# zeal-up/ORB_SLAM_Tracking

Hardware: AMD Instinct MI355X
Metric: frames/sec (extract+match, 1000 feat, 640x480) (higher is better)
Workload: dtype u8

## Files before the change

### include/orbx.h

```cpp
#ifndef ORBX_H_
#define ORBX_H_

#include <stddef.h>
#include <stdint.h>

#ifdef __cplusplus
extern "C" {
#endif

#define ORBX_OK 0
#define ORBX_E_EMPTY (-1)
#define ORBX_E_BADARG (-2)
#define ORBX_E_TOOSMALL (-3)
#define ORBX_MAX_FRAME_DIM 4096
#define ORBX_E_HIP (-4)
#define ORBX_E_CAPACITY (-5)
#define ORBX_E_RCCL (-6)

typedef struct orbx_keypoint {
  float x, y, size, angle, response;
  int32_t octave, class_id;
} orbx_keypoint;

typedef struct orbx_params {
// ... 607 lines not shown
                                      const float* d_map_normals, const float* d_map_dist, const uint8_t* d_map_desc32,
                                      const uint8_t* d_map_mask, const float* d_pose, const float* K, const orbx_bounds* bounds,
                                      float th, float nnratio, int32_t* d_matches, const uint8_t* d_outlier, uint8_t* d_point_view,
                                      orbx_local_result* d_res);
int orbx_match_local_map(orbx_ctx* ctx, const orbx_keypoint* kps_un, const uint8_t* desc32, int n, int map_n,
                         const float* map_points, const float* map_normals, const float* map_dist, const uint8_t* map_desc32,
                         const uint8_t* map_mask, const float* pose, const float* K, const orbx_bounds* bounds, float th,
                         float nnratio, int32_t* matches, const uint8_t* outlier, uint8_t* point_view, orbx_local_result* res);

#define ORBX_KFPROJ_BAD_INPUT 2
#define ORBX_KFPROJ_NONFINITE 4
typedef struct orbx_kfproj_result {
  int32_t status;
  int32_t nmatches;
  int32_t n_points;
  int32_t n_found;
  int32_t n_behind_kept;
  int32_t n_out_image;
  int32_t n_out_distance;
  int32_t n_with_candidates;
  int32_t n_over_dist;
  int32_t n_displaced;
  int32_t n_rot_removed;
  int32_t n_outliers_cleared;
  int32_t rounds;
} orbx_kfproj_result;

int orbx_match_keyframe_projection_batch_device(orbx_ctx* ctx, int n_frames, int n_pairs, const int32_t* h_kf, const int32_t* h_cur,
                                                const int32_t* h_point_set, const orbx_keypoint* d_kps_un, const uint8_t* d_desc32,
                                                const int32_t* d_n, int capacity, int n_point_sets, const float* d_points,
                                                const uint8_t* d_point_mask, const uint8_t* d_point_desc32, const float* d_point_dist,
                                                const float* d_pose, const float* K, const orbx_bounds* bounds, float th, int orb_dist,
                                                int check_orientation, int32_t* d_matches, const uint8_t* d_outlier,
                                                orbx_kfproj_result* d_res);
int orbx_match_keyframe_projection(orbx_ctx* ctx, const orbx_keypoint* kf_kps_un, const uint8_t* kf_desc32, int kf_n,
                                   const orbx_keypoint* cur_kps_un, const uint8_t* cur_desc32, int cur_n, const float* points,
                                   const uint8_t* mask, const uint8_t* point_desc32, const float* point_dist, const float* pose,
                                   const float* K, const orbx_bounds* bounds, float th, int orb_dist, int check_orientation,
                                   int32_t* matches, const uint8_t* outlier, orbx_kfproj_result* res);

#define ORBX_MSIM3_BAD_INPUT 2
#define ORBX_MSIM3_NONFINITE 4
typedef struct orbx_msim3_result {
  int32_t status;
  int32_t n_found;
  int32_t n_points_12;
  int32_t n_behind_12;
  int32_t n_out_image_12;
  int32_t n_out_distance_12;
  int32_t n_with_candidates_12;
  int32_t n_over_dist_12;
  int32_t n_points_21, n_behind_21, n_out_image_21, n_out_distance_21, n_with_candidates_21, n_over_dist_21;
  int32_t n_one_sided;
  int32_t reserved;
} orbx_msim3_result;

int orbx_match_sim3_batch_device(orbx_ctx* ctx, int n_frames, int n_pairs, const int32_t* h_kf1, const int32_t* h_kf2,
                                 const int32_t* h_set1, const int32_t* h_set2, const orbx_keypoint* d_kps_un, const uint8_t* d_desc32,
                                 const int32_t* d_n, int capacity, int n_point_sets, const float* d_points,
                                 const uint8_t* d_point_mask, const uint8_t* d_point_desc32, const float* d_point_dist,
                                 const float* d_pose, const float* d_sim3, const float* K, const orbx_bounds* bounds, float th,
                                 int orb_dist, int32_t* d_matches, orbx_msim3_result* d_res);
int orbx_match_sim3(orbx_ctx* ctx, const orbx_keypoint* kps_un1, const uint8_t* desc1, int n1, const float* points1,
                    const uint8_t* mask1, const uint8_t* point_desc1, const float* point_dist1, const float* pose1,
                    const orbx_keypoint* kps_un2, const uint8_t* desc2, int n2, const float* points2, const uint8_t* mask2,
                    const uint8_t* point_desc2, const float* point_dist2, const float* pose2, const float* sim3, const float* K,
                    const orbx_bounds* bounds, float th, int orb_dist, int32_t* matches12, orbx_msim3_result* res);

#define ORBX_TRI_BAD_INPUT 2
#define ORBX_TRI_NONFINITE 4
#define ORBX_TRI_LOW_BASELINE 8
#define ORBX_TRI_ZERO_BASELINE 16
typedef struct orbx_tri_match_result {
  int32_t status;
  int32_t nmatches;
  int32_t n_queries;
  int32_t n_with_candidates;
  int32_t n_epipole_rejected;
  int32_t n_epiline_rejected;
  int32_t n_rot_removed;
  float baseline, ex, ey;
  float F12[9];
} orbx_tri_match_result;

int orbx_match_triangulation_batch_device(orbx_ctx* ctx, int n_frames, int n_pairs, const int32_t* h_kf1, const int32_t* h_kf2,
                                          const orbx_keypoint* d_kps_un, const uint8_t* d_desc32, const int32_t* d_n, int capacity,
                                          const uint32_t* d_fv_node, const uint32_t* d_fv_feat, const int32_t* d_fv_n,
                                          const uint8_t* d_mask, const float* d_pose, const float* K, const float* d_median_depth,
                                          int check_orientation, int32_t* d_matches12, orbx_tri_match_result* d_res);
int orbx_match_triangulation(orbx_ctx* ctx, const orbx_keypoint* kps_un1, const uint8_t* desc1, int n1, const uint32_t* fv_node1,
                             const uint32_t* fv_feat1, int fv_n1, const uint8_t* mask1, const float* pose1,
                             const orbx_keypoint* kps_un2, const uint8_t* desc2, int n2, const uint32_t* fv_node2,
                             const uint32_t* fv_feat2, int fv_n2, const uint8_t* mask2, const float* pose2, const float* K,
                             float median_depth2, int check_orientation, int32_t* matches12, orbx_tri_match_result* res);

typedef struct orbx_tri_result {
  int32_t status;
  int32_t n_matches;
  int32_t n_points;
  int32_t n_low_parallax, n_w_zero, n_behind_1, n_behind_2, n_reproj_1, n_reproj_2, n_zero_dist, n_scale;
} orbx_tri_result;

int orbx_triangulate_matches_batch_device(orbx_ctx* ctx, int n_frames, int n_pairs, const int32_t* h_kf1, const int32_t* h_kf2,
                                          const orbx_keypoint* d_kps_un, const int32_t* d_n, int capacity, const float* d_pose,
                                          const float* K, const int32_t* d_matches12, float* d_points, uint8_t* d_point_mask,
                                          float* d_point_normal, float* d_point_dist, orbx_tri_result* d_res);
int orbx_triangulate_matches(orbx_ctx* ctx, const orbx_keypoint* kps_un1, int n1, const float* pose1, const orbx_keypoint* kps_un2,
                             int n2, const float* pose2, const float* K, const int32_t* matches12, float* points, uint8_t* point_mask,
                             float* point_normal, float* point_dist, orbx_tri_result* res);

#define ORBX_STAGE_PYRAMID 0
#define ORBX_STAGE_FAST 1
#define ORBX_STAGE_SELECT 2
#define ORBX_STAGE_DESCRIBE 3
#define ORBX_STAGE_MATCH 4
#define ORBX_STAGE_COUNT 5
int orbx_profile_enable(orbx_ctx* ctx, int on);
int orbx_profile_stages(orbx_ctx* ctx, unsigned stage_mask);
int orbx_profile_reset(orbx_ctx* ctx);
int orbx_profile_get(orbx_ctx* ctx, double* ms, int64_t* launches);

typedef struct orbx_multi orbx_multi;
int orbx_multi_create(const orbx_params* params, int n_devices, const int* device_ids, int max_width, int max_height,
                      int max_batch_per_device, orbx_multi** out);
void orbx_multi_destroy(orbx_multi* m);
int orbx_multi_size(const orbx_multi* m);
orbx_ctx* orbx_multi_ctx(orbx_multi* m, int r);
const char* orbx_multi_last_error(const orbx_multi* m);
int orbx_multi_shard_range(int n_frames, int n_devices, int r, int* lo, int* hi);
int orbx_multi_extract_match_batch_device(orbx_multi* m, int n_frames, const uint8_t* const* d_imgs, int width, int height, int stride,
                                          size_t frame_stride_bytes, orbx_keypoint* const* d_kps, uint8_t* const* d_desc32, int capacity,
                                          int32_t* const* d_n_out, const orbx_bounds* bounds, int window_size, float nnratio,
                                          int check_orientation, int32_t* const* d_matches12, int32_t* const* d_nmatches,
                                          int32_t* counts_all);

int orbx_multi_set_pipeline_depth(orbx_multi* m, int depth);
int orbx_multi_extract_match_batch_device_async(orbx_multi* m, int n_frames, const uint8_t* const* d_imgs, int width, int height,
                                                int stride, size_t frame_stride_bytes, orbx_keypoint* const* d_kps,
                                                uint8_t* const* d_desc32, int capacity, int32_t* const* d_n_out,
                                                const orbx_bounds* bounds, int window_size, float nnratio, int check_orientation,
                                                int32_t* const* d_matches12, int32_t* const* d_nmatches, int32_t* counts_all);
int orbx_multi_wait_one(orbx_multi* m);
int orbx_multi_wait(orbx_multi* m);

int orbx_debug_candidates(orbx_ctx* ctx, int frame, int level, float* xyr, int cap);
int orbx_debug_selection_units(orbx_ctx* ctx, int frame, int32_t* counts, int32_t* redone);
int orbx_debug_distribute_device(orbx_ctx* ctx, const float* xyr, int n, int min_x, int max_x, int min_y, int max_y,
                                 int n_features, int variant, float* out_xyr, int cap);
int orbx_debug_std_sort(orbx_ctx* ctx, int32_t* triples, int n);
int orbx_debug_sincos(orbx_ctx* ctx, const float* angle_deg, int n, float* cos_out, float* sin_out);

int orbx_debug_last_launch(const orbx_ctx* ctx, int32_t* info8);
int orbx_debug_pyr_cols(int groups, int two_groups, uint32_t* info5);
int orbx_debug_match_counters(orbx_ctx* ctx, uint32_t* info4);
int orbx_debug_set(const char* key, long long value);
int orbx_debug_path_codes(int width, int height, int n, const int32_t* xs, const int32_t* ys, uint64_t* from_tables,
                          uint64_t* from_walk);

#ifdef __cplusplus
}
#endif
#endif
```

### orb_slam_tracking_amd/__init__.py

```python
from __future__ import annotations

import collections
import contextlib
import ctypes
import os
from typing import Optional, Sequence, Tuple

import numpy as np

__all__ = ["KEYPOINT_DTYPE", "OrbxError", "ORBextractor", "ORBmatcher", "Frame", "lib", "lib_path",
           "HFResult", "HF_RESULT_DTYPE", "Vocabulary", "BowResult", "BOW_MAX_FEATURES", "Database", "DB_MAX_RESULTS", "debug_database_shape", "InitResult", "INIT_RESULT_DTYPE", "BAResult", "BA_RESULT_DTYPE", "BA_SKIPPED", "BA_BAD_INPUT", "BA_NONFINITE", "BA_FEW_POINTS", "BA_NEGATIVE_DEPTH", "PoseResult", "POSE_RESULT_DTYPE", "POSE_BAD_INPUT", "POSE_NONFINITE", "POSE_FEW_POINTS", "PnpResult", "PNP_RESULT_DTYPE", "PNP_BAD_INPUT", "PNP_NONFINITE", "PNP_FEW_POINTS", "PNP_BAD_DRAWS", "PNP_NO_POSE", "PNP_RAND_MAX", "PnPsolver", "sample_pnp_draws", "Sim3Result", "SIM3_RESULT_DTYPE", "SIM3_BAD_INPUT", "SIM3_NONFINITE", "SIM3_FEW_POINTS", "SIM3_BAD_DRAWS", "SIM3_NO_RESULT", "Sim3Solver", "sample_sim3_draws", "MatchSim3Result", "MSIM3_RESULT_DTYPE", "MSIM3_BAD_INPUT", "MSIM3_NONFINITE", "ProjResult", "PROJ_RESULT_DTYPE", "PROJ_BAD_INPUT", "PROJ_NONFINITE", "LocalResult", "LOCAL_RESULT_DTYPE", "LOCAL_BAD_INPUT", "LOCAL_NONFINITE", "LOCAL_NOT_IN_VIEW", "LOCAL_SEEN", "KfProjResult", "KFPROJ_RESULT_DTYPE", "KFPROJ_BAD_INPUT", "KFPROJ_NONFINITE", "TriMatchResult", "TRI_MATCH_RESULT_DTYPE", "TriResult", "TRI_RESULT_DTYPE", "TRI_BAD_INPUT", "TRI_NONFINITE", "TRI_LOW_BASELINE", "TRI_ZERO_BASELINE", "Optimizer", "sample_sets", "INIT_TOO_FEW_MATCHES", "INIT_BAD_SETS", "INIT_NO_SCORE", "INIT_BAD_MATCHES",
           "STAGES", "E_EMPTY", "E_BADARG", "E_TOOSMALL", "E_HIP", "E_CAPACITY", "E_RCCL",
           "Sim3OptResult", "SIM3OPT_RESULT_DTYPE", "SIM3OPT_BAD_INPUT", "SIM3OPT_NONFINITE",
           "MatchScwResult", "SCW_RESULT_DTYPE", "SCW_BAD_INPUT", "SCW_NONFINITE", "SCW_TAKEN_UNMAPPED", "loop_accepted",
           "MapFuser", "FuseResult", "FUSE_RESULT_DTYPE", "FUSE_BAD_INPUT", "FUSE_NONFINITE", "FUSE_OCCUPIED_UNMAPPED", "FUSE_NONE",
           "FUSE_ADD", "FUSE_KEEP_OCCUPANT", "FUSE_REPLACE_OCCUPANT", "FUSE_BAD_OCCUPANT",
           "LbaResult", "LBA_RESULT_DTYPE", "LBA_BAD_INPUT", "LBA_NONFINITE", "LBA_MAX_FREE",
           "MapResult", "MAP_RESULT_DTYPE", "MAP_RESULT_FIELDS", "MAP_NORMALS", "MAP_DESCRIPTORS", "MAP_BAD_INPUT", "MAP_NONFINITE"]

from ._records import (KEYPOINT_DTYPE, _Params, _Bounds, _Camera, _Stats, HFResult, HF_RESULT_DTYPE, InitResult,
                       INIT_RESULT_DTYPE, BAResult, BA_RESULT_DTYPE, PoseResult, POSE_RESULT_DTYPE, PnpResult, PNP_RESULT_DTYPE,
                       Sim3Result, SIM3_RESULT_DTYPE, Sim3OptResult, SIM3OPT_RESULT_DTYPE, ProjResult, PROJ_RESULT_DTYPE,
                       PROJ_RESULT_FIELDS, LocalResult, LOCAL_RESULT_DTYPE, LOCAL_RESULT_FIELDS, MatchScwResult, SCW_RESULT_DTYPE,
                       SCW_RESULT_FIELDS, KfProjResult, KFPROJ_RESULT_DTYPE, KFPROJ_RESULT_FIELDS, MatchSim3Result,
# ... 131 lines not shown
    L.orbx_get_scale_factor.restype = f32
    L.orbx_get_tables.argtypes = [vp, vp, vp, vp, vp, vp]
    L.orbx_get_umax.argtypes = [vp, vp]
    L.orbx_extract.argtypes = [vp, vp, i32, i32, i32, i32, i32, vp, vp, i32, vp]
    L.orbx_host_register.argtypes = [vp, vp, sz]
    L.orbx_host_unregister.argtypes = [vp, vp]
    L.orbx_extract_batch.argtypes = [vp, i32, vp, i32, i32, i32, sz, i32, i32, vp, vp, i32, vp, vp]
    L.orbx_extract_batch_device.argtypes = [vp, i32, vp, i32, i32, i32, sz, vp, vp, i32, vp]
    L.orbx_level_size.argtypes = [vp, i32, vp, vp]
    L.orbx_download_pyramid.argtypes = [vp, i32, i32, i32, vp, i32]
    L.orbx_match_init.argtypes = [vp, vp, vp, i32, vp, vp, i32, ctypes.POINTER(_Bounds), i32, f32, i32, vp,
                                  ctypes.POINTER(ctypes.c_int32), ctypes.POINTER(_Stats)]
    L.orbx_match_init_batch_device.argtypes = [vp, i32, vp, vp, vp, vp, vp, i32, ctypes.POINTER(_Bounds), i32, f32, i32,
                                               vp, vp, vp]
    L.orbx_extract_match_batch_device.argtypes = [vp, i32, vp, i32, i32, i32, sz, vp, vp, i32, vp, i32, vp, vp,
                                                  ctypes.POINTER(_Bounds), i32, f32, i32, vp, vp, vp]
    L.orbx_extract_match_batch_device_async.argtypes = [vp, i32, vp, i32, i32, i32, sz, vp, vp, i32, vp, i32, vp, vp,
                                                  ctypes.POINTER(_Bounds), i32, f32, i32, vp, vp, vp]
    L.orbx_extract_match_batch_host_async.argtypes = L.orbx_extract_match_batch_device_async.argtypes
    L.orbx_set_opencv_variant.argtypes = [vp, i32, i32]
    L.orbx_set_libm_variant.argtypes = [vp, i32]
    L.orbx_set_pipeline_depth.argtypes = [vp, i32]
    L.orbx_wait_one.argtypes = [vp]
    L.orbx_wait.argtypes = [vp]
    L.orbx_order_after.argtypes = [vp, vp]
    L.orbx_order_before.argtypes = [vp, vp]
    L.orbx_profile_stages.argtypes = [vp, ctypes.c_uint]
    L.orbx_undistort_keypoints.argtypes = [vp, vp, i32, ctypes.POINTER(_Camera), vp]
    L.orbx_undistort_batch_device.argtypes = [vp, i32, vp, vp, i32, ctypes.POINTER(_Camera), vp]
    L.orbx_image_bounds.argtypes = [vp, ctypes.POINTER(_Camera), i32, i32, ctypes.POINTER(_Bounds)]
    L.orbx_to_gray.argtypes = [vp, vp, i32, i32, i32, i32, i32, vp, i32]
    L.orbx_to_gray_batch_device.argtypes = [vp, i32, vp, i32, i32, i32, sz, i32, i32, vp, i32, sz]
    L.orbx_check_homography.argtypes = [vp, i32, vp, vp, vp, i32, vp, i32, vp, f32, vp, vp, vp, vp]
    L.orbx_check_fundamental.argtypes = [vp, i32, vp, vp, i32, vp, i32, vp, f32, vp, vp, vp, vp]
    L.orbx_check_rt.argtypes = [vp, i32, vp, vp, vp, vp, i32, vp, i32, vp, vp, f32, vp, vp, vp, vp]
    L.orbx_find_models_batch_device.argtypes = [vp, i32, i32, vp, vp, vp, vp, i32, vp, i32, vp, f32, vp, vp, vp, vp]
    L.orbx_find_models.argtypes = [vp, vp, i32, vp, i32, vp, i32, vp, f32, ctypes.POINTER(HFResult), vp, vp, vp]
    L.orbx_initialize_batch_device.argtypes = [vp, i32, i32, vp, vp, vp, vp, i32, vp, i32, vp, vp, f32, f32, i32, vp, vp, vp]
    L.orbx_initialize.argtypes = [vp, vp, i32, vp, i32, vp, i32, vp, vp, f32, f32, i32, ctypes.POINTER(InitResult), vp, vp]
    L.orbx_bundle_adjust_batch_device.argtypes = [vp, i32, i32, vp, vp, vp, vp, i32, vp, vp, vp, vp, vp, vp, i32, i32, i32, vp, vp]
    L.orbx_bundle_adjust.argtypes = [vp, vp, i32, vp, i32, vp, vp, vp, vp, vp, vp, i32, i32, i32, ctypes.POINTER(BAResult), vp]
    L.orbx_pose_optimize_batch_device.argtypes = [vp, i32, i32, vp, vp, vp, vp, i32, vp, i32, vp, vp, vp, vp, vp, i32, vp, vp]
    L.orbx_pose_optimize.argtypes = [vp, vp, i32, vp, vp, vp, vp, vp, i32, ctypes.POINTER(PoseResult), vp]
    f64 = ctypes.c_double
    L.orbx_pnp_ransac_table.argtypes = [f64, i32, i32, f32, i32, vp]
    L.orbx_pnp_solve_batch_device.argtypes = [vp, i32, i32, vp, vp, vp, vp, i32, vp, i32, vp, vp, vp, vp, f64, i32, i32, f32, f32, i32,
                                              vp, vp, vp, vp, vp]
    L.orbx_pnp_solve.argtypes = [vp, vp, i32, vp, vp, vp, vp, f64, i32, i32, f32, f32, i32, vp, ctypes.POINTER(PnpResult), vp]
    L.orbx_sim3_ransac_table.argtypes = [f64, i32, i32, i32, vp]
    L.orbx_sim3_solve_batch_device.argtypes = [vp, i32, i32, vp, vp, vp, vp, vp, vp, i32, vp, i32, vp, vp, vp, vp, vp, i32, f64, i32, i32,
                                               f32, i32, vp, vp, vp, vp, vp]
    L.orbx_match_sim3_batch_device.argtypes = [vp, i32, i32, vp, vp, vp, vp, vp, vp, vp, i32, i32, vp, vp, vp, vp, vp, vp, vp,
                                               ctypes.POINTER(_Bounds), f32, i32, vp, vp]
    L.orbx_match_sim3.argtypes = [vp, vp, vp, i32, vp, vp, vp, vp, vp, vp, vp, i32, vp, vp, vp, vp, vp, vp, vp, ctypes.POINTER(_Bounds),
                                  f32, i32, vp, ctypes.POINTER(MatchSim3Result)]
    L.orbx_sim3_solve.argtypes = [vp, vp, i32, vp, vp, vp, vp, i32, vp, vp, vp, vp, vp, vp, i32, f64, i32, i32, f32, i32, vp,
                                  ctypes.POINTER(Sim3Result), vp, vp, vp]
    L.orbx_optimize_sim3_batch_device.argtypes = [vp, i32, i32, vp, vp, vp, vp, vp, vp, i32, vp, i32, vp, vp, vp, vp, vp, vp, i32, f32,
                                                  i32, i32, vp, vp]
    L.orbx_optimize_sim3.argtypes = [vp, vp, i32, vp, vp, vp, vp, i32, vp, vp, vp, vp, vp, vp, vp, i32, f32, i32, i32,
                                     ctypes.POINTER(Sim3OptResult), vp]
    L.orbx_match_scw_batch_device.argtypes = [vp, i32, i32, vp, vp, vp, vp, vp, i32, i32, i32, vp, vp, vp, vp, vp, vp, vp, vp,
                                              ctypes.POINTER(_Bounds), f32, i32, vp, vp, vp]
    L.orbx_match_scw.argtypes = [vp, vp, vp, i32, i32, vp, vp, vp, vp, vp, vp, vp, ctypes.POINTER(_Bounds), f32, i32, vp, vp, i32,
                                 ctypes.POINTER(MatchScwResult)]
    L.orbx_sim3_compose_scw_batch_device.argtypes = [vp, i32, i32, vp, vp, vp, vp]
    L.orbx_sim3_compose_scw.argtypes = [vp, vp, vp, vp]
    L.orbx_fuse_batch_device.argtypes = [vp, i32, i32, vp, vp, vp, vp, vp, i32, i32, i32, vp, vp, vp, vp, vp, vp, vp, vp, vp,
                                         ctypes.POINTER(_Bounds), f32, i32, vp, vp, vp, vp, vp, vp]
    L.orbx_fuse_scw_batch_device.argtypes = [vp, i32, i32, vp, vp, vp, vp, vp, i32, i32, i32, vp, vp, vp, vp, vp, vp, vp, vp,
                                             ctypes.POINTER(_Bounds), f32, i32, vp, vp, vp, vp, vp, vp]
    L.orbx_fuse.argtypes = [vp, vp, vp, i32, i32, vp, vp, vp, vp, vp, vp, vp, vp, ctypes.POINTER(_Bounds), f32, i32, vp, vp, vp, vp, vp,
                            ctypes.POINTER(FuseResult)]
    L.orbx_fuse_scw.argtypes = [vp, vp, vp, i32, i32, vp, vp, vp, vp, vp, vp, vp, ctypes.POINTER(_Bounds), f32, i32, vp, vp, vp, vp, vp,
                                ctypes.POINTER(FuseResult)]
    L.orbx_local_ba_batch_device.argtypes = [vp, i32, i32, vp, vp, vp, vp, i32, vp, vp, vp, i32, vp, vp, i32, i32, vp, vp, vp, vp, vp, i32, i32,
                                             vp, vp, vp, vp]
    L.orbx_local_ba.argtypes = [vp, i32, i32, vp, vp, i32, vp, vp, i32, vp, vp, vp, vp, i32, i32, vp, vp, vp, ctypes.POINTER(LbaResult)]
    L.orbx_debug_local_ba_lds_max_free.argtypes = [i32]
    L.orbx_map_update_batch_device.argtypes = [vp, i32, i32, vp, vp, vp, vp, i32, vp, vp, vp, vp, i32, vp, vp, vp, i32, i32, vp, vp, vp, vp, vp,
                                               i32, vp, vp, vp, vp, vp]
    L.orbx_map_update.argtypes = [vp, i32, i32, vp, vp, vp, i32, vp, vp, vp, i32, vp, vp, vp, vp, i32, vp, vp, vp, vp, ctypes.POINTER(MapResult)]
    L.orbx_vocabulary_parse_text.argtypes = [ctypes.c_char_p, vp, vp, vp, vp, vp, vp, i32]
    L.orbx_vocabulary_create.argtypes = [vp, i32, i32, i32, i32, i32, vp, vp, vp, vp, ctypes.POINTER(vp)]
    L.orbx_vocabulary_load_text.argtypes = [vp, ctypes.c_char_p, ctypes.POINTER(vp)]
    L.orbx_vocabulary_destroy.argtypes = [vp]
    L.orbx_vocabulary_destroy.restype = None
    L.orbx_vocabulary_info.argtypes = [vp, vp]
    L.orbx_vocabulary_get_nodes.argtypes = [vp, vp, vp, vp, vp, i32]
    L.orbx_vocabulary_save_text.argtypes = [vp, ctypes.c_char_p, i32]
    L.orbx_vocabulary_train_device.argtypes = [vp, i32, i32, i32, i32, ctypes.c_uint64, i32, i32, vp, vp, i32, ctypes.POINTER(vp), vp, vp]
    L.orbx_vocabulary_train.argtypes = [vp, i32, i32, i32, i32, ctypes.c_uint64, i32, i32, vp, vp, ctypes.POINTER(vp), vp, vp]
    L.orbx_debug_voc_train_seed_grid_min.argtypes = [ctypes.c_longlong]
    L.orbx_bow_transform_batch_device.argtypes = [vp, vp, i32, vp, vp, i32, i32, vp, vp, vp, vp, vp, vp, vp]
    L.orbx_bow_transform.argtypes = [vp, vp, vp, i32, i32, vp, vp, vp, vp, vp, vp, vp]
    L.orbx_bow_score_batch_device.argtypes = [vp, vp, i32, i32, vp, vp, vp, vp, vp, i32, vp]
    L.orbx_bow_score.argtypes = [vp, vp, vp, vp, i32, vp, vp, i32, vp]
    L.orbx_match_bow_batch_device.argtypes = [vp, i32, i32, vp, vp, vp, vp, vp, i32, vp, vp, vp, vp, f32, i32, vp, vp]
    L.orbx_match_bow.argtypes = [vp, vp, vp, i32, vp, vp, i32, vp, vp, i32, vp, vp, i32, vp, f32, i32, vp, vp]
    L.orbx_match_projection_batch_device.argtypes = [vp, i32, i32, vp, vp, vp, vp, vp, vp, i32, i32, vp, vp, vp, vp, vp, vp,
                                                     ctypes.POINTER(_Bounds), f32, i32, vp, vp]
    L.orbx_match_projection.argtypes = [vp, vp, vp, i32, vp, vp, i32, vp, vp, vp, vp, vp, vp, ctypes.POINTER(_Bounds), f32, i32, vp,
                                        ctypes.POINTER(ProjResult)]
    L.orbx_match_local_map_batch_device.argtypes = [vp, i32, i32, vp, vp, vp, vp, vp, i32, i32, i32, vp, vp, vp, vp, vp, vp, vp, vp,
                                                    ctypes.POINTER(_Bounds), f32, f32, vp, vp, vp, vp]
    L.orbx_match_local_map.argtypes = [vp, vp, vp, i32, i32, vp, vp, vp, vp, vp, vp, vp, ctypes.POINTER(_Bounds), f32, f32, vp, vp, vp,
                                       ctypes.POINTER(LocalResult)]
    L.orbx_match_keyframe_projection_batch_device.argtypes = [vp, i32, i32, vp, vp, vp, vp, vp, vp, i32, i32, vp, vp, vp, vp, vp, vp,
                                                              ctypes.POINTER(_Bounds), f32, i32, i32, vp, vp, vp]
    L.orbx_match_keyframe_projection.argtypes = [vp, vp, vp, i32, vp, vp, i32, vp, vp, vp, vp, vp, vp, ctypes.POINTER(_Bounds), f32,
                                                 i32, i32, vp, vp, ctypes.POINTER(KfProjResult)]
    L.orbx_match_triangulation_batch_device.argtypes = [vp, i32, i32, vp, vp, vp, vp, vp, i32, vp, vp, vp, vp, vp, vp, vp, i32, vp, vp]
    L.orbx_match_triangulation.argtypes = [vp, vp, vp, i32, vp, vp, i32, vp, vp, vp, vp, i32, vp, vp, i32, vp, vp, vp, f32, i32, vp,
                                           ctypes.POINTER(TriMatchResult)]
    L.orbx_triangulate_matches_batch_device.argtypes = [vp, i32, i32, vp, vp, vp, vp, i32, vp, vp, vp, vp, vp, vp, vp, vp]
    L.orbx_triangulate_matches.argtypes = [vp, vp, i32, vp, vp, i32, vp, vp, vp, vp, vp, vp, vp, ctypes.POINTER(TriResult)]
    L.orbx_database_create.argtypes = [vp, vp, ctypes.POINTER(vp)]
    L.orbx_database_destroy.argtypes = [vp]
    L.orbx_database_destroy.restype = None
    L.orbx_database_clear.argtypes = [vp]
    L.orbx_database_size.argtypes = [vp]
    L.orbx_database_add_batch_device.argtypes = [vp, vp, i32, vp, vp, vp, i32, vp]
    L.orbx_database_query_batch_device.argtypes = [vp, vp, i32, vp, vp, vp, i32, i32, i32, vp, vp, vp]
    L.orbx_database_add.argtypes = [vp, vp, vp, vp, i32, vp]
    L.orbx_database_query.argtypes = [vp, vp, vp, vp, i32, i32, i32, vp, vp, vp]
    L.orbx_database_get_inverted_file.argtypes = [vp, vp, vp, vp, ctypes.c_int64]
    L.orbx_database_get_inverted_file.restype = ctypes.c_int64
    L.orbx_debug_database_shape.argtypes = [i32, i32]
    L.orbx_multi_create.argtypes = [ctypes.POINTER(_Params), i32, vp, i32, i32, i32, ctypes.POINTER(vp)]
    L.orbx_multi_destroy.argtypes = [vp]
    L.orbx_multi_destroy.restype = None
    L.orbx_multi_size.argtypes = [vp]
    L.orbx_multi_ctx.argtypes = [vp, i32]
    L.orbx_multi_ctx.restype = vp
    L.orbx_multi_last_error.argtypes = [vp]
    L.orbx_multi_last_error.restype = ctypes.c_char_p
    L.orbx_multi_shard_range.argtypes = [i32, i32, i32, ctypes.POINTER(i32), ctypes.POINTER(i32)]
    L.orbx_multi_extract_match_batch_device.argtypes = [vp, i32, vp, i32, i32, i32, sz, vp, vp, i32, vp, ctypes.POINTER(_Bounds), i32,
                                                        f32, i32, vp, vp, vp]
    L.orbx_multi_extract_match_batch_device_async.argtypes = L.orbx_multi_extract_match_batch_device.argtypes
    L.orbx_multi_set_pipeline_depth.argtypes = [vp, i32]
    L.orbx_multi_wait_one.argtypes = [vp]
    L.orbx_multi_wait.argtypes = [vp]
    L.orbx_profile_enable.argtypes = [vp, i32]
    L.orbx_profile_reset.argtypes = [vp]
    L.orbx_profile_get.argtypes = [vp, vp, vp]
    L.orbx_debug_candidates.argtypes = [vp, i32, i32, vp, i32]
    L.orbx_debug_distribute_device.argtypes = [vp, vp, i32, i32, i32, i32, i32, i32, i32, vp, i32]
    L.orbx_debug_std_sort.argtypes = [vp, vp, i32]
    L.orbx_debug_sincos.argtypes = [vp, vp, i32, vp, vp]
    L.orbx_debug_set.argtypes = [ctypes.c_char_p, ctypes.c_longlong]
    L.orbx_debug_last_launch.argtypes = [vp, vp]
    L.orbx_debug_pyr_cols.argtypes = [ctypes.c_int, ctypes.c_int, vp]
    L.orbx_debug_match_counters.argtypes = [vp, vp]
    L.orbx_debug_selection_units.argtypes = [vp, i32, vp, vp]
    L.orbx_debug_path_codes.argtypes = [ctypes.c_int, ctypes.c_int, ctypes.c_int, vp, vp, vp, vp]
    _LIB = L
    for name in KNOBS:
        v = os.environ.get("ORBX_" + name.upper())
        if v is not None:
            debug_set(name, _knob_value(name, v))
    return L


KNOBS = ("no_bands", "pyr_bands", "pyr_strips", "bands_min_frames", "no_split", "lat_trace", "fast_wg_max_cells", "match_no_general",
         "match_no_mfma", "oct_big_depth", "oct_big_no_fallback", "multi_force_rccl")
KNOB_UNSET = -(1 << 63)


def _knob_value(name: str, text: str) -> int:
    try:
        return int(text)
    except ValueError:
        return 1


def debug_set(name: str, value: Optional[int]) -> None:
    r = lib().orbx_debug_set(name.encode(), KNOB_UNSET if value is None else int(value))
    if r != 0:
        raise OrbxError(r, "orbx_debug_set(%r)" % name)


@contextlib.contextmanager
def knobs(**values: Optional[int]):
    try:
        for name, value in values.items():
            debug_set(name, value)
        yield
    finally:
        for name in values:
            debug_set(name, None)


def _ptr(a) -> ctypes.c_void_p:
    if a is None:
        return ctypes.c_void_p(0)
    if isinstance(a, np.ndarray):
        return ctypes.c_void_p(a.ctypes.data)
    if hasattr(a, "data_ptr"):
        return ctypes.c_void_p(a.data_ptr())
    return ctypes.c_void_p(int(a))


def _nbytes(a):
    if isinstance(a, np.ndarray):
        return int(a.nbytes)
    if hasattr(a, "data_ptr") and hasattr(a, "numel"):
        return int(a.numel()) * int(a.element_size())
    return None


def _need(what: str, a, nbytes: int) -> None:
    have = _nbytes(a)
    if have is not None and have < nbytes:
        raise ValueError("%s holds %d bytes, the call needs %d" % (what, have, nbytes))


def _pair_lists(names, lists, n_frames: Optional[int] = None, n_sets: Optional[int] = None, set_what: str = "") -> list:
    rows = [np.ascontiguousarray(a, np.int32).reshape(-1) for a in lists]
    n = len(rows[0])
    for r in rows:
        if len(r) != n:
            raise OrbxError(E_BADARG, "%s and %s must have the same length" % (", ".join(names[:-1]), names[-1]))
    if n and (n_frames is not None or n_sets is not None):
        top = [int(r.view(np.uint32).max()) for r in rows]
        if n_frames is not None and max(top if n_sets is None else top[:-1]) >= n_frames:
            raise ValueError("a pair names a frame outside the batch of %d" % n_frames)
        if n_sets is not None and top[-1] >= n_sets:
            raise ValueError("a pair names a %s outside the %d given" % (set_what, n_sets))
    return rows


def _k9(K) -> np.ndarray:
    return np.ascontiguousarray(K, np.float32).reshape(9)


def _bounds(bounds) -> _Bounds:
    return _Bounds(*[int(v) for v in bounds])


def _keys(keys) -> np.ndarray:
    return np.ascontiguousarray(keys, KEYPOINT_DTYPE).reshape(-1)


def _desc(desc, n: Optional[int] = None, message: str = "") -> Optional[np.ndarray]:
    if desc is None and n is not None:
        return None
    d = np.ascontiguousarray(desc, np.uint8).reshape(-1, 32)
    if n is not None and len(d) != n:
        raise OrbxError(E_BADARG, message)
    return d


def _points(points, width: int = 3) -> np.ndarray:
    return np.ascontiguousarray(points, np.float32).reshape(-1, width)


def _flags(flags, n: int, message: str) -> Optional[np.ndarray]:
    if flags is None:
        return None
    f = np.ascontiguousarray(np.asarray(flags) != 0, np.uint8).reshape(-1)
    if len(f) != n:
        raise OrbxError(E_BADARG, message)
    return f


def _row(row, n: int, message: str) -> np.ndarray:
    out = np.full(max(n, 1), -1, np.int32)
    if row is not None:
        given = np.asarray(row, np.int32).reshape(-1)
        if len(given) != n:
            raise OrbxError(E_BADARG, message)
        out[:n] = given
    return out


def _per_level(table, nlevels: int, name: str) -> Optional[np.ndarray]:
    t = None if table is None else np.ascontiguousarray(table, np.float32)
    if t is not None and len(t) != nlevels:
        raise OrbxError(E_BADARG, "%s must have one entry per pyramid level" % name)
    return t


def _pose12(Tcw) -> np.ndarray:
    T = np.asarray(Tcw, np.float32)
    if T.ndim == 1:
        return np.ascontiguousarray(T.reshape(12))
    return np.ascontiguousarray(np.r_[T[:3, :3].reshape(9), T[:3, 3]], np.float32)


def _camera_K(K, holder, who: str, what: str = "frame") -> np.ndarray:
    if K is not None:
        return K
    cam = getattr(holder, "camera", None)
    if cam is None:
        raise OrbxError(E_BADARG, "%s needs K (the %s carries no camera)" % (who, what))
    return np.array([[cam[0], 0, cam[2]], [0, cam[1], cam[3]], [0, 0, 1]], np.float32)


def _need_batch(imgs, n_frames, width, height, stride, frame_stride, kps, desc, n, capacity, first=None, second=None, matches12=None,
                nmatches=None, stats=None, init_res=None, p3d=None, triangulated=None, ba_res=None, p3d_out=None) -> None:
    if n_frames > 0 and imgs is not None:
        _need("the frames", imgs, (n_frames - 1) * frame_stride + (height - 1) * stride + width)
    _need("the keypoint array", kps, n_frames * capacity * 28)
    _need("the descriptor array", desc, n_frames * capacity * 32)
    _need("the count array", n, n_frames * 4)
# ... 1907 lines not shown
```

### orb_slam_tracking_amd/csrc/orbx_api.cpp

```cpp
#include <hip/hip_runtime.h>

#include <algorithm>
#include <cmath>
#include <cstdio>
#include <cstring>
#include <ctime>
#include <string>
#include <vector>

#include "orbx_host.h"
#include "orbx_knobs.h"

namespace orbx {

std::atomic<long long> g_knob[KNOB_COUNT] = {
#define ORBX_KNOB_INIT(e, n) {KNOB_UNSET},
    ORBX_KNOB_LIST(ORBX_KNOB_INIT)
#undef ORBX_KNOB_INIT
};

namespace {

inline int cvRoundF(float v) { return (int)lrintf(v); }
inline int cvRoundD(double v) { return (int)lrint(v); }

}
}

using namespace orbx;

struct PyrTabInfo {
  int32_t xoff[ORBX_MAX_LEVELS], yoff[ORBX_MAX_LEVELS];
  int ok, dual2;
};

struct SizedBufs {
  DeviceBuf<uint8_t> dPyr;
  DeviceBuf<uint32_t> dCand;
  DeviceBuf<int> dCandCount;
  DeviceBuf<int> dCellCount;
  DeviceBuf<int> dMaxN;
  PinnedBuf<int> hMaxN;
  DeviceBuf<ResizeTab> dTab;
  DeviceBuf<FastCell> dCells;
  DeviceBuf<SelKp> dSel;
  DeviceBuf<int> dNsel;
  DeviceBuf<SelKp> dSelStage;
  DeviceBuf<int> dNselLevel;
  DeviceBuf<uint8_t> dOctScratch;
  DeviceBuf<uint32_t> dOctTab;
  DeviceBuf<PyrTileRect> dPyrTiles;
  DeviceBuf<PyrTileTap> dPyrTaps;
  DeviceBuf<uint8_t> dIn;
  DeviceBuf<orbx_keypoint> dKps;
  DeviceBuf<uint8_t> dDesc;
  PinnedBuf<int> hNsel;
  PinnedBuf<int> hFlags;
  PinnedBuf<int> hWide;
  PinnedBuf<orbx_keypoint> hKpsPin;
  PinnedBuf<uint8_t> hDescPin;
};

struct PairBlock {
  orbx_keypoint* kps = nullptr;
  uint8_t* desc = nullptr;
  int32_t* n = nullptr;
  size_t bytes = 0;
  PairBlock() = default;
  PairBlock(void* base, size_t cap) {
    Layout L(base);
    kps = L.take<orbx_keypoint>(2 * cap);
    desc = L.take<uint8_t>(2 * cap * 32);
    n = L.take<int32_t>(2);
    bytes = L.size();
  }
};

struct orbx_ctx {
  orbx_params p{};
  int device = 0;
  hipStream_t st = nullptr;
  bool ownStream = false;
  int maxW = 0, maxH = 0, maxB = 0;
  std::vector<float> scale, invScale, sigma2, invSigma2;
  std::vector<int> quota;
  int umax[16]{};
  int gaussVariant = 0, grayVariant = 0;
  int libmVariant = ORBX_LIBM_DEFAULT;
  int selCap = 0;

  int curW = 0, curH = 0, curStride0 = 0;
  Geom g{};
  std::vector<ResizeTab> hTab;

  SizedBufs bufs;
  size_t pyrBytes = 0;
  size_t candEntries = 0;
  int candHintL[ORBX_MAX_LEVELS]{};
  int maxSlotsUsed = 0;
  size_t cellCountEntries = 0;
  size_t tabEntries = 0;
  PyrTabInfo pyrInfo{};
  std::vector<FastCell> hCells;
  size_t cellEntries = 0;
  int fastWaveOk = 0;
  OctLaunch oct{};
  int maxQuota = 0;
  size_t pyrTileCap = 0;
  std::vector<PyrTileRect> hPyrTiles;
  std::vector<PyrTileTap> hPyrTaps;
  int nPyrTiles = 0, pyrTileBuf0 = 0, pyrTileBuf = 0;
  size_t octTabEntries = 0;
  std::vector<uint32_t> hOctTab;
  size_t octScratchBytes = 0;
  bool wideExpected = false;
  int wideIdle = 0;
  bool wideLaunched[2]{};
  bool eventOrdered = false;
  int lastLaunch[8]{};
  struct LateMatch {
    bool valid = false;
    int nPairs = 0, capacity = 0, window = 0, checkOri = 0;
    float nnratio = 0;
    orbx_bounds b{};
    const orbx_keypoint* dKps = nullptr;
    const uint8_t* dDesc = nullptr;
    const int* dN = nullptr;
    int32_t* dMatches12 = nullptr;
    int32_t* dNmatches = nullptr;
    int32_t* dStats = nullptr;
  } late[2];
  size_t inBytes = 0;
  int pinFrames = 0;
  DeviceBuf<int> dMatchScratch;
  DeviceBuf<unsigned int> dMatchDiag;
  HeldArray<int32_t> pairs;
  DeviceBuf<uint8_t> dMblk;
  PinnedBuf<uint8_t> hMblk;
  PairBlock dM, hM;
  PinnedBuf<int> hMo;
  DeviceBuf<int> dMi;
  size_t mCap = 0;
  DeviceBuf<uint8_t> io;
  InitScratch init;
  DeviceBuf<uint8_t> dColor;
  MatchBowScratch matchBow;
  BaScratch ba;
  PoseScratch pose;
  PnpScratch pnp;
  Sim3Scratch sim3;
  Sim3OptScratch sim3Opt;
  LbaScratch lba;
  MapScratch map;
  TriScratch tri;

  const uint8_t* lastImg0 = nullptr;
  long long lastFrameStride0 = 0;
  int lastB = 0;

  hipStream_t st2 = nullptr;
  hipEvent_t evFork = nullptr, evJoin = nullptr;
  hipEvent_t evOrder = nullptr;

  unsigned profMask = 0;
  hipEvent_t ev[2][2][ORBX_STAGE_COUNT][2]{};
  bool used[2][2][ORBX_STAGE_COUNT]{};
  hipEvent_t evDone[2]{};
  hipEvent_t evDone2[2]{};
  bool done2Used[2]{};
  std::vector<orbx_ctx*> lanes;
  unsigned laneIssue = 0, laneDone = 0;
  bool noSplit = false;
  DeviceBuf<uint8_t> dPipeOut;
  hipEvent_t evOut[2]{};
  bool outUsed[2]{};
  bool hostInput = false;
  unsigned seqIssue = 0;
  int pending = 0;
  int parity = 0;
  double ms[ORBX_STAGE_COUNT]{};
  int64_t launches[ORBX_STAGE_COUNT]{};

  std::string err;
};

namespace {

void computeTables(orbx_ctx* c) {
  const int nl = c->p.nlevels;
  const double scaleFactor = (double)c->p.scale_factor;
  c->scale.assign(nl, 1.f);
  c->sigma2.assign(nl, 1.f);
  c->invScale.assign(nl, 1.f);
  c->invSigma2.assign(nl, 1.f);
  for (int i = 1; i < nl; i++) {
    c->scale[i] = (float)(c->scale[i - 1] * scaleFactor);
    c->sigma2[i] = c->scale[i] * c->scale[i];
  }
  for (int i = 0; i < nl; i++) {
    c->invScale[i] = 1.0f / c->scale[i];
    c->invSigma2[i] = 1.0f / c->sigma2[i];
  }
  c->quota.assign(nl, 0);
  const float factor = (float)(1.0f / scaleFactor);
  const float powv = c->libmVariant ? powf(factor, (float)nl) : (float)std::pow((double)factor, (double)(float)nl);
  float desired = c->p.nfeatures * (1 - factor) / (1 - powv);
  int sum = 0;
  for (int l = 0; l < nl - 1; l++) {
    c->quota[l] = cvRoundF(desired);
    sum += c->quota[l];
    desired *= factor;
  }
  c->quota[nl - 1] = std::max(c->p.nfeatures - sum, 0);
  c->selCap = 0;
  for (int q : c->quota) c->selCap += q;
  const int HALF = 15;
  const int vmax = (int)std::floor(HALF * std::sqrt(2.f) / 2 + 1);
  const int vmin = (int)std::ceil(HALF * std::sqrt(2.f) / 2);
  const double hp2 = HALF * HALF;
  for (int v = 0; v <= HALF; v++) c->umax[v] = 0;
  for (int v = 0; v <= vmax; ++v) c->umax[v] = cvRoundD(std::sqrt(hp2 - v * v));
  for (int v = HALF, v0 = 0; v >= vmin; --v) {
    while (c->umax[v0] == c->umax[v0 + 1]) ++v0;
    c->umax[v] = v0;
    ++v0;
  }
}

void levelSize(const orbx_ctx* c, int w, int h, int l, int* lw, int* lh) {
  *lw = cvRoundF(w * c->invScale[l]);
  *lh = cvRoundF(h * c->invScale[l]);
}

void appendPyrTables(const Geom& g, std::vector<ResizeTab>* tab, PyrTabInfo* info) {
  static_assert(sizeof(ResizeTab) == 8 && sizeof(PyrXGroup) == 8 * sizeof(ResizeTab) && sizeof(PyrYRow) == 2 * sizeof(ResizeTab), "table units");
  *info = PyrTabInfo{};
  info->ok = g.nlevels > 1;
  for (int l = 1; l < g.nlevels; l++) {
    const LevelGeom& S = g.L[l - 1];
    const LevelGeom& D = g.L[l];
    const int sw = S.w, sh = S.h, ng = (D.w + 3) / 4;
    if (sw < 8 || D.h >= 32768 || D.w > 4096) info->ok = 0;
    if (tab->size() & 1) tab->push_back(ResizeTab{0, 0});
    info->xoff[l] = (int32_t)(tab->size() / 2);
    const int lim = (sw - 1) & ~3;
    for (int gx = 0; gx < ng; gx++) {
      PyrXGroup x{};
      const ResizeTab* e = tab->data() + D.xtabOff + 4 * gx;
      const int base = e[0].ofs & ~3;
      x.o[0] = (uint32_t)base;
      x.o[1] = (uint32_t)std::min(base + 4, lim);
      x.o[2] = (uint32_t)std::min(base + 8, lim);
      const uint32_t zero = 0x0c0c0c0cu;
      for (int i = 0; i < 4; i++) {
        const int k = e[i].ofs - base, c0 = e[i].coef & 0xffff, c1 = (int)((uint32_t)e[i].coef >> 16);
        const int k1 = c1 ? k + 1 : k;
        if (k < 0 || k1 > 11 || c0 + c1 > 2048) { info->ok = 0; continue; }
        const bool second = k1 > 7;
        if (second && k < 4) { info->ok = 0; continue; }
        const uint32_t sel = 0x0c000c00u | (uint32_t)(second ? k - 4 : k) | ((uint32_t)(second ? k1 - 4 : k1) << 16);
        if (i < 2) {
          if (second) info->ok = 0;
          x.sel[i] = sel;
        } else if (i == 2) {
          x.sel[2] = second ? zero : sel;
          x.sel[3] = second ? sel : zero;
          if (second) info->dual2 = 1;
        } else {
          x.sel[4] = second ? zero : sel;
          x.sel[5] = second ? sel : zero;
        }
        x.cf[i] = ((uint32_t)c0 << 4) | (((uint32_t)c1 << 4) << 16);
      }
      ResizeTab raw[8];
      memcpy(raw, &x, sizeof(x));
      tab->insert(tab->end(), raw, raw + 8);
    }
    info->yoff[l] = (int32_t)(tab->size() / 2);
    for (int dy = 0; dy < D.h; dy++) {
      const ResizeTab t = (*tab)[D.ytabOff + dy];
      const int sy0 = std::min(std::max(t.ofs, 0), sh - 1), sy1 = std::min(std::max(t.ofs + 1, 0), sh - 1);
      const int c0 = t.coef & 0xffff, c1 = (int)((uint32_t)t.coef >> 16);
      if (c0 + c1 > 2048) info->ok = 0;
      const PyrYRow y{(uint32_t)sy0 * (uint32_t)S.stride, (uint32_t)sy1 * (uint32_t)S.stride, (uint32_t)c0 << 8, (uint32_t)c1 << 8};
      ResizeTab raw[2];
      memcpy(raw, &y, sizeof(y));
      tab->insert(tab->end(), raw, raw + 2);
    }
  }
}

int buildGeometry(orbx_ctx* c, int w, int h, int stride0, Geom* out, std::vector<ResizeTab>* tab, PyrTabInfo* pyrInfo = nullptr) {
  Geom g{};
  g.nlevels = c->p.nlevels;
  g.iniTh = std::min(std::max(c->p.ini_th_fast, 0), 255);
  g.minTh = std::min(std::max(c->p.min_th_fast, 0), 255);
  g.selCap = c->selCap;
  int cellBase = 0;
  int64_t pyrOff = 0, candOff = 0;
  int tabOff = 0;
  if (tab) tab->clear();
  int pw = 0, ph = 0;
  for (int l = 0; l < g.nlevels; l++) {
    LevelGeom& L = g.L[l];
    levelSize(c, w, h, l, &L.w, &L.h);
    if (L.w > ORBX_MAX_FRAME_DIM || L.h > ORBX_MAX_FRAME_DIM) {
      c->err = "frame larger than ORBX_MAX_FRAME_DIM (4096) pixels in width or height";
      return ORBX_E_BADARG;
    }
    L.maxBX = L.w - ORBX_EDGE + 3;
    L.maxBY = L.h - ORBX_EDGE + 3;
    const float width = (float)(L.maxBX - ORBX_MIN_BORDER), height = (float)(L.maxBY - ORBX_MIN_BORDER);
    if (width < 35.f || height < 35.f) return ORBX_E_TOOSMALL;
    if ((int)std::round(width / height) < 1) return ORBX_E_TOOSMALL;
    L.nCols = (int)(width / 35.f);
    L.nRows = (int)(height / 35.f);
    L.wCell = (int)std::ceil(width / L.nCols);
    L.hCell = (int)std::ceil(height / L.nRows);
    L.cellBase = cellBase;
    L.colsInv24 = L.nCols > 0 ? (uint32_t)(((1u << 24) + (uint32_t)L.nCols - 1u) / (uint32_t)L.nCols) : 0u;
    cellBase += L.nCols * L.nRows;
    int cap = 0;
    for (int i = 0; i < L.nRows; i++) {
      const int iniY = ORBX_MIN_BORDER + i * L.hCell;
      if (iniY >= L.maxBY - 3) continue;
      const int ch = std::min(iniY + L.hCell + 6, L.maxBY) - iniY;
      for (int j = 0; j < L.nCols; j++) {
        const int iniX = ORBX_MIN_BORDER + j * L.wCell;
        if (iniX >= L.maxBX - 6) continue;
        const int cw = std::min(iniX + L.wCell + 6, L.maxBX) - iniX;
        if (cw < 7 || ch < 7) continue;
        cap += ((cw - 6 + 1) / 2) * ((ch - 6 + 1) / 2);
      }
    }
    L.candMax = std::max(cap, 1);
    L.segCap = alignUp(std::max(((L.wCell + 1) / 2) * ((L.hCell + 1) / 2), 1), 4);
    L.candCap = L.nCols * L.nRows * L.segCap;
    L.candOff = candOff;
    candOff += (int64_t)L.candCap * c->maxB;
    L.quota = c->quota[l];
    L.scale = c->scale[l];
    L.patchSize = (int)(31 * c->scale[l]);
    if (l == 0) {
      L.stride = stride0;
      L.imgOff = 0;
      L.frameStride = 0;
      L.xtabOff = L.ytabOff = 0;
    } else {
      L.stride = alignUp(L.w, 64);
      L.imgOff = pyrOff;
      L.frameStride = (int64_t)L.stride * L.h;
      pyrOff += L.frameStride * c->maxB;
      if (tab) {
        const int sw = pw, sh = ph, dw = L.w, dh = L.h;
        const double scale_x = 1.0 / ((double)dw / sw), scale_y = 1.0 / ((double)dh / sh);
        L.xtabOff = tabOff;
        const int dwPad = alignUp(dw, 4);
        for (int dx = 0; dx < dwPad; dx++) {
          const int d = std::min(dx, dw - 1);
          float fx = (float)((d + 0.5) * scale_x - 0.5);
          int sx = (int)std::floor(fx);
          fx -= sx;
          if (sx < 0) { fx = 0; sx = 0; }
          if (sx >= sw - 1) { fx = 0; sx = sw - 1; }
          const int c0 = cvRoundF((1.f - fx) * 2048), c1 = cvRoundF(fx * 2048);
          tab->push_back(ResizeTab{sx, (c0 & 0xffff) | (c1 << 16)});
        }
        int span = 0;
        for (int dx = 0; dx + 3 < dwPad; dx += 4)
          span = std::max(span, (*tab)[L.xtabOff + dx + 3].ofs - (*tab)[L.xtabOff + dx].ofs);
        L.resizeSpanOk = span <= 7 ? 1 : 0;
        tabOff += dwPad;
        L.ytabOff = tabOff;
        for (int dy = 0; dy < dh; dy++) {
          float fy = (float)((dy + 0.5) * scale_y - 0.5);
          int sy = (int)std::floor(fy);
          fy -= sy;
          const int c0 = cvRoundF((1.f - fy) * 2048), c1 = cvRoundF(fy * 2048);
          tab->push_back(ResizeTab{sy, (c0 & 0xffff) | (c1 << 16)});
        }
        tabOff += dh;
      }
    }
    pw = L.w;
    ph = L.h;
  }
  g.nCellsTotal = cellBase;
  if (tab) {
    PyrTabInfo info;
    appendPyrTables(g, tab, &info);
    if (pyrInfo) *pyrInfo = info;
  }
  *out = g;
  return ORBX_OK;
}

int buildFastCells(const Geom& g, std::vector<FastCell>* out) {
  out->assign((size_t)g.nCellsTotal, FastCell{});
  bool ok = true, narrow = true;
  for (int l = 0; l < g.nlevels; l++) {
    const LevelGeom& L = g.L[l];
    for (int ci = 0; ci < L.nRows; ci++)
      for (int cj = 0; cj < L.nCols; cj++) {
        const int local = ci * L.nCols + cj;
        FastCell& c = (*out)[(size_t)L.cellBase + local];
        c.xoff_level = (uint32_t)l << 16;
        c.stride = (uint32_t)L.stride;
        c.segOff = (uint32_t)local * (uint32_t)L.segCap;
        c.segCap = (uint32_t)L.segCap;
        const int iniY = ORBX_MIN_BORDER + ci * L.hCell, iniX = ORBX_MIN_BORDER + cj * L.wCell;
        if (iniY >= L.maxBY - 3 || iniX >= L.maxBX - 6) continue;
        const int maxY = std::min(iniY + L.hCell + 6, L.maxBY), maxX = std::min(iniX + L.wCell + 6, L.maxBX);
        const int cw = maxX - iniX, ch = maxY - iniY;
        if (cw < 7 || ch < 7) continue;
        const int ax0 = iniX & ~3, xoff = iniX - ax0, nw = (maxX - ax0 + 3) >> 2;
        if (nw > 16 || ch > 64) ok = false;
        if (nw > 12) narrow = false;
        c.imgOff = (uint32_t)(iniY * L.stride + ax0);
        c.nw_ch = (uint32_t)nw | ((uint32_t)ch << 16);
        c.iw_ih = (uint32_t)(cw - 6) | ((uint32_t)(ch - 6) << 16);
        c.xoff_level |= (uint32_t)xoff;
        c.ox_oy = ((uint32_t)(cj * L.wCell - xoff) & 0xffffu) | ((uint32_t)(ci * L.hCell) << 16);
      }
  }
  return ok ? (narrow ? 2 : 1) : 0;
}

struct Sizes {
  size_t pyrBytes, candEntries, tabEntries;
};
Sizes sizesOf(const orbx_ctx* c, const Geom& g, size_t tabEntries) {
  Sizes s{};
  const LevelGeom& last = g.L[g.nlevels - 1];
  s.pyrBytes = g.nlevels > 1 ? (size_t)(last.imgOff + last.frameStride * c->maxB) : 0;
  s.candEntries = (size_t)(last.candOff + (int64_t)last.candCap * c->maxB);
  s.tabEntries = tabEntries;
  return s;
}

int octDepthBits(int height, float hX) {
  int e = std::max((int)std::ceil(hX) + 1, height), d = 0;
  while (e > 1) { e = (e + 1) >> 1; d++; }
  return std::max(d, 1);
}

constexpr long long kPyrTilesMaxPixels = 2500000ll;
void pyrTileGrid(const Geom& g, int* TX, int* TY) {
  *TX = std::max(1, (g.L[1].w + 35) / 36);
  *TY = std::max(1, (g.L[1].h + 27) / 28);
}
bool buildPyrTiles(const Geom& g, const std::vector<ResizeTab>& tab, std::vector<PyrTileRect>* out, std::vector<PyrTileTap>* taps,
                   int* nTiles, int* buf0Bytes, int* bufBytes) {
  const int nl = g.nlevels;
  *nTiles = 0;
  *buf0Bytes = *bufBytes = 0;
  out->clear();
  taps->clear();
  if (nl < 2 || g.L[0].w > 32000 || g.L[0].h > 32000) return false;
  int TX, TY;
  pyrTileGrid(g, &TX, &TY);
  out->assign((size_t)TX * TY * nl, PyrTileRect{});
  taps->assign((size_t)TX * TY * ORBX_PYR_TILE_TAPS, PyrTileTap{0, 0});
  int maxPix = 0, maxPix0 = 0;
  for (int tj = 0; tj < TY; tj++)
    for (int ti = 0; ti < TX; ti++) {
      PyrTileRect* R = out->data() + (size_t)(tj * TX + ti) * nl;
      for (int l = 1; l < nl; l++) {
        R[l].ox0 = (int16_t)((long long)ti * g.L[l].w / TX); R[l].ox1 = (int16_t)((long long)(ti + 1) * g.L[l].w / TX);
        R[l].oy0 = (int16_t)((long long)tj * g.L[l].h / TY); R[l].oy1 = (int16_t)((long long)(tj + 1) * g.L[l].h / TY);
      }
      for (int l = nl - 1; l >= 0; l--) {
        int x0 = R[l].ox0, x1 = R[l].ox1, y0 = R[l].oy0, y1 = R[l].oy1;
        const bool ownEmpty = x1 <= x0 || y1 <= y0;
        if (l + 1 < nl && R[l + 1].nx1 > R[l + 1].nx0 && R[l + 1].ny1 > R[l + 1].ny0) {
          const ResizeTab* xt = tab.data() + g.L[l + 1].xtabOff;
          const ResizeTab* yt = tab.data() + g.L[l + 1].ytabOff;
          const int w = g.L[l].w, h = g.L[l].h;
          const int fx0 = std::min(std::max(xt[R[l + 1].nx0].ofs, 0), w - 1), fx1 = std::min(xt[R[l + 1].nx1 - 1].ofs + 1, w - 1) + 1;
          const int fy0 = std::min(std::max(yt[R[l + 1].ny0].ofs, 0), h - 1);
          const int fy1 = std::min(std::max(yt[R[l + 1].ny1 - 1].ofs + 1, 0), h - 1) + 1;
          if (ownEmpty) { x0 = fx0; x1 = fx1; y0 = fy0; y1 = fy1; }
          else { x0 = std::min(x0, fx0); x1 = std::max(x1, fx1); y0 = std::min(y0, fy0); y1 = std::max(y1, fy1); }
        } else if (ownEmpty) {
          x0 = x1 = y0 = y1 = 0;
        }
        R[l].nx0 = (int16_t)x0; R[l].nx1 = (int16_t)x1; R[l].ny0 = (int16_t)y0; R[l].ny1 = (int16_t)y1;
        (l == 0 ? maxPix0 : maxPix) = std::max(l == 0 ? maxPix0 : maxPix, (x1 - x0) * (y1 - y0));
        if ((long long)(x1 - x0) * (y1 - y0) * (x1 - x0) >= (1ll << 20)) { out->clear(); taps->clear(); return false; }
      }
      PyrTileTap* T = taps->data() + (size_t)(tj * TX + ti) * ORBX_PYR_TILE_TAPS;
      int nT = 0;
      for (int l = 1; l < nl; l++) {
        const ResizeTab* xt = tab.data() + g.L[l].xtabOff;
        const ResizeTab* yt = tab.data() + g.L[l].ytabOff;
        const int sw = g.L[l - 1].w, sh = g.L[l - 1].h;
        const int nw = R[l].nx1 - R[l].nx0, nh = R[l].ny1 - R[l].ny0;
        if (nT + nw + nh > ORBX_PYR_TILE_TAPS) { out->clear(); taps->clear(); return false; }
        for (int x = R[l].nx0; x < R[l].nx1; x++) {
          const int sx = xt[x].ofs, sx1 = std::min(sx + 1, sw - 1);
          T[nT++] = PyrTileTap{(uint32_t)(sx - R[l - 1].nx0) | ((uint32_t)(sx1 - sx) << 16), (uint32_t)xt[x].coef};
        }
        for (int y = R[l].ny0; y < R[l].ny1; y++) {
          const int sy0 = std::min(std::max(yt[y].ofs, 0), sh - 1), sy1 = std::min(std::max(yt[y].ofs + 1, 0), sh - 1);
          T[nT++] = PyrTileTap{(uint32_t)(sy0 - R[l - 1].ny0) | ((uint32_t)(sy1 - sy0) << 16), (uint32_t)yt[y].coef};
        }
      }
    }
  const int buf0 = (maxPix0 + 63) & ~63, buf = (maxPix + 63) & ~63;
  if (buf0 <= 0 || buf <= 0 || ORBX_PYR_TILE_TAPS * (int)sizeof(PyrTileTap) + buf0 + 2 * buf > 60 * 1024) { out->clear(); taps->clear(); return false; }
  *nTiles = TX * TY;
  *buf0Bytes = buf0;
  *bufBytes = buf;
  return true;
}

void octCodeTable(const OctLevel& O, uint32_t* out) {
  for (int xi = 0; xi < O.tabW; xi++) {
    const float x = (float)xi;
    int root = (int)(x / O.hX);
    root = std::min(std::max(root, 0), O.nIni - 1);
    int ul = (int)(O.hX * (float)root), br = (int)(O.hX * (float)(root + 1));
    uint32_t s = 0;
    for (int d = 0; d < 16; d++) {
      const int mid = ul + ((br - ul + 1) >> 1);
      const uint32_t q = !(x < (float)mid);
      if (q) ul = mid; else br = mid;
      s = (s << 2) | q;
    }
    out[2 * xi] = s;
    out[2 * xi + 1] = (uint32_t)root;
  }
  uint32_t* ty = out + 2 * (size_t)O.tabW;
  for (int yi = 0; yi < O.tabH; yi++) {
    const float y = (float)yi;
    int ul = 0, br = O.height;
    uint32_t s = 0;
    for (int d = 0; d < 16; d++) {
      const int mid = ul + ((br - ul + 1) >> 1);
      const uint32_t q = !(y < (float)mid);
      if (q) ul = mid; else br = mid;
      s = (s << 2) | (q << 1);
    }
    ty[yi] = s;
  }
}
void octBigPlan(OctLevel* O, int nMax) {
  O->bigDMax = -1;
  O->bigD0 = 0; O->bigBuckets = 0; O->bigCapB = 0;
  if (O->nIni < 1 || O->nIni > ORBX_OCTB_MAX_BUCKETS || O->quota < 1) return;
  int kq = 0;
  while ((long long)O->nIni << (2 * (kq + 1)) <= (long long)O->quota && kq < 8) kq++;
  int d = kq;
  while (d > 0 && ((long long)O->nIni << (2 * d)) > ORBX_OCTB_MAX_BUCKETS) d--;
  O->bigDMax = d;
  octBigChoose(O, nMax, 0);
}
inline size_t octBigTabDwords(const OctLevel& O) {
  return O.bigDMax >= 0 ? ((size_t)O.nIni << O.bigDMax) + 1 + ((size_t)1 << O.bigDMax) + 1 : 0;
}
size_t octTabLayout(OctLaunch* P) {
  size_t off = 0;
  for (int l = 0; l < P->nlevels; l++) {
    OctLevel& O = P->lev[l];
    O.tabOff = (int32_t)off;
    off += (2 * (size_t)O.tabW + (size_t)O.tabH + 1) & ~(size_t)1;
    O.bigTabOff = (int32_t)off;
    off += (octBigTabDwords(O) + 1) & ~(size_t)1;
  }
  return off;
}
bool octBigTable(const OctLevel& O, const uint32_t* codeTab, uint32_t* out) {
  const int d0 = O.bigDMax, nx = O.nIni << d0, ny = 1 << d0;
  auto topBits = [&](uint32_t s, int odd) {
    uint32_t v = 0;
    for (int d = 1; d <= d0; d++) v = (v << 1) | ((s >> (2 * (16 - d) + odd)) & 1u);
    return v;
  };
  std::vector<int> first((size_t)std::max(nx, ny) + 1);
// ... 1511 lines not shown

int orbx_debug_selection_units(orbx_ctx* ctx, int frame, int32_t* counts, int32_t* redone) {
  if (!ctx || frame < 0 || frame >= ctx->lastB || !counts) return ORBX_E_BADARG;
  if (hipSetDevice(ctx->device) != hipSuccess) return ORBX_E_HIP;
  {
    const int w = waitAll(ctx);
    if (w == ORBX_E_HIP) return w;
  }
  const int nl = ctx->p.nlevels;
  std::vector<int32_t> raw((size_t)nl);
  HIPCHK(hipMemcpy(raw.data(), ctx->bufs.dNselLevel + (size_t)frame * nl, sizeof(int32_t) * (size_t)nl, hipMemcpyDeviceToHost));
  for (int l = 0; l < nl; l++) {
    counts[l] = raw[l] < 0 ? raw[l] : (raw[l] & ~ORBX_OCT_REDONE);
    if (redone) redone[l] = raw[l] >= 0 && (raw[l] & ORBX_OCT_REDONE) ? 1 : 0;
  }
  return ORBX_OK;
}

}

extern "C" {

int orbx_debug_distribute_device(orbx_ctx* ctx, const float* xyr, int n, int min_x, int max_x, int min_y, int max_y,
                                 int n_features, int variant, float* out_xyr, int cap) {
  if (!ctx || n < 0 || (n > 0 && !xyr) || max_x <= min_x || max_y <= min_y || n_features < 0 || n > ORBX_OCT_MAX_CAND)
    return ORBX_E_BADARG;
  if (hipSetDevice(ctx->device) != hipSuccess) return ORBX_E_HIP;
  OctLaunch P{};
  P.nlevels = 1;
  P.selStride = std::max(n_features, 1);
  OctLevel& O = P.lev[0];
  O.width = max_x - min_x;
  O.height = max_y - min_y;
  O.nIni = (int)std::round((float)O.width / (float)O.height);
  if (O.nIni < 1 || O.nIni > 255) return ORBX_E_TOOSMALL;
  O.hX = (float)O.width / (float)O.nIni;
  O.depthBits = octDepthBits(O.height, O.hX);
  O.tabW = O.tabH = 4096;
  O.wCell = O.hCell = 1 << 20;
  O.nCols = 1;
  O.quota = n_features;
  O.cellBase = 0; O.nCells = 1; O.segCap = alignUp(std::max(n, 1), 4);
  P.nCellsTotal = 1;
  P.candCap[0] = std::max(n, 1);
  P.scrNMax[0] = std::min(std::max(8 * n, 16384), ORBX_OCT_MAX_CAND);
  P.scrStride[0] = (int64_t)octScratchBytes(P.scrNMax[0], std::max(n_features, O.nIni));
  std::vector<uint32_t> packed((size_t)alignUp(std::max(n, 1), 4));
  for (int i = 0; i < n; i++) {
    const int x = (int)xyr[3 * i], y = (int)xyr[3 * i + 1], r = (int)xyr[3 * i + 2];
    if (x < 0 || x > 4095 || y < 0 || y > 4095 || r < 0 || r > 255) return ORBX_E_BADARG;
    packed[i] = packCand(x, y, r);
  }
  O.tabW = std::max(O.tabW, O.width);
  O.tabH = std::max(O.tabH, O.height);
  octBigPlan(&O, P.scrNMax[0]);
  octTabLayout(&P);
  std::vector<uint32_t> codeTab;
  octCodeTables(&P, &codeTab);
  std::vector<SelKp> sel(std::max(n_features, 1));
  int res[2] = {0, 0};
  DeviceBuf<uint32_t> dC, dT;
  DeviceBuf<int> dI;
  DeviceBuf<SelKp> dS;
  DeviceBuf<uint8_t> dScr;
  HIPCHK(dC.grow(packed.size() * 4));
  HIPCHK(dI.grow(2 * sizeof(int)));
  HIPCHK(dS.grow(sel.size() * sizeof(SelKp)));
  HIPCHK(dScr.grow((size_t)P.scrStride[0]));
  HIPCHK(dT.grow(codeTab.size() * 4));
  P.codeTab = dT;
  HIPCHK(hipMemcpyAsync(dT, codeTab.data(), codeTab.size() * 4, hipMemcpyHostToDevice, ctx->st));
  HIPCHK(hipMemcpyAsync(dC, packed.data(), packed.size() * 4, hipMemcpyHostToDevice, ctx->st));
  int hi[2] = {n, -7};
  HIPCHK(hipMemcpyAsync(dI, hi, sizeof hi, hipMemcpyHostToDevice, ctx->st));
  const int hintN[ORBX_MAX_LEVELS] = {n};
  HIPCHK(launch_octree(ctx->st, 1, dC, dI, P, dS, dI + 1, dScr, nullptr, variant == 5 ? hintN : nullptr,
                       variant == 1 ? -1 : variant == 2 ? 1024 : variant == 3 ? 512 : variant == 4 ? (2048 | 0x10000) : variant == 5 ? -2 :
                       variant == 6 ? -3 : 0, nullptr));
  HIPCHK(hipMemcpyAsync(res, dI, sizeof res, hipMemcpyDeviceToHost, ctx->st));
  HIPCHK(hipMemcpyAsync(sel.data(), dS, sel.size() * sizeof(SelKp), hipMemcpyDeviceToHost, ctx->st));
  HIPCHK(hipStreamSynchronize(ctx->st));
  if (res[1] < 0) return ORBX_E_CAPACITY;
  res[1] &= ~0x40000000;
  for (int i = 0; i < res[1] && i < cap; i++) {
    out_xyr[3 * i] = (float)(sel[i].x - ORBX_MIN_BORDER);
    out_xyr[3 * i + 1] = (float)(sel[i].y - ORBX_MIN_BORDER);
    out_xyr[3 * i + 2] = (float)sel[i].response;
  }
  return res[1];
}

int orbx_debug_path_codes(int width, int height, int n, const int32_t* xs, const int32_t* ys, uint64_t* from_tables,
                          uint64_t* from_walk) {
  if (width <= 0 || height <= 0 || width > 4096 || height > 4096 || n < 0 || (n > 0 && (!xs || !ys || !from_tables || !from_walk)))
    return ORBX_E_BADARG;
  OctLevel O{};
  O.width = width;
  O.height = height;
  O.nIni = (int)std::round((float)width / (float)height);
  if (O.nIni < 1 || O.nIni > 255) return ORBX_E_TOOSMALL;
  O.hX = (float)width / (float)O.nIni;
  O.tabW = width;
  O.tabH = height;
  std::vector<uint32_t> tab((size_t)2 * width + height + 2);
  octCodeTable(O, tab.data());
  for (int i = 0; i < n; i++) {
    const int xi = xs[i], yi = ys[i];
    if (xi < 0 || xi >= width || yi < 0 || yi >= height) return ORBX_E_BADARG;
    from_tables[i] = ((uint64_t)tab[2 * (size_t)xi + 1] << 32) | (uint64_t)(tab[2 * (size_t)xi] | tab[2 * (size_t)width + yi]);
    const float x = (float)xi, y = (float)yi;
    int root = (int)(x / O.hX);
    root = std::min(std::max(root, 0), O.nIni - 1);
    int ulx = (int)(O.hX * (float)root), brx = (int)(O.hX * (float)(root + 1)), uly = 0, bry = height;
    uint64_t code = (uint64_t)root;
    for (int d = 0; d < 16; d++) {
      const int midX = ulx + ((brx - ulx + 1) >> 1), midY = uly + ((bry - uly + 1) >> 1);
      const int qx = !(x < (float)midX), qy = !(y < (float)midY);
      if (qx) ulx = midX; else brx = midX;
      if (qy) uly = midY; else bry = midY;
      code = (code << 2) | (uint64_t)(qy * 2 + qx);
    }
    from_walk[i] = code;
  }
  return ORBX_OK;
}

int orbx_debug_set(const char* key, long long value) {
  static const char* const names[KNOB_COUNT] = {
#define ORBX_KNOB_NAME(e, n) n,
      ORBX_KNOB_LIST(ORBX_KNOB_NAME)
#undef ORBX_KNOB_NAME
  };
  if (!key) return ORBX_E_BADARG;
  for (int k = 0; k < KNOB_COUNT; k++)
    if (std::strcmp(key, names[k]) == 0) {
      g_knob[k].store(value, std::memory_order_relaxed);
      return ORBX_OK;
    }
  return ORBX_E_BADARG;
}

int orbx_debug_pyr_cols(int groups, int two_groups, uint32_t* info5) {
  if (!info5 || groups < 1 || groups > (two_groups ? 2 : 1) * ORBX_PYR_THREADS) return ORBX_E_BADARG;
  uint32_t c[2];
  pyrColsOf(groups, two_groups != 0, c);
  info5[0] = (c[0] >> 31) + 1;
  info5[1] = (c[0] >> 20 & 0x1ffu) + 1;
  info5[2] = (c[1] >> 20 & 0x1ffu) + 1;
  info5[3] = c[0] & 0xfffffu;
  info5[4] = c[1] & 0xfffffu;
  return ORBX_OK;
}

int orbx_debug_last_launch(const orbx_ctx* ctx, int32_t* info8) {
  if (!ctx || !info8) return ORBX_E_BADARG;
  for (int i = 0; i < 8; i++) info8[i] = ctx->lastLaunch[i];
  return ORBX_OK;
}

int orbx_debug_match_counters(orbx_ctx* ctx, uint32_t* info4) {
  if (!ctx || !info4) return ORBX_E_BADARG;
  for (int i = 0; i < 4; i++) info4[i] = 0;
  if (!ctx->dMatchDiag) return ORBX_OK;
  if (hipSetDevice(ctx->device) != hipSuccess) return ORBX_E_HIP;
  const int w = waitAll(ctx);
  if (w != ORBX_OK) return w;
  HIPCHK(hipStreamSynchronize(ctx->st));
  HIPCHK(hipMemcpy(info4, ctx->dMatchDiag, 4 * sizeof(uint32_t), hipMemcpyDeviceToHost));
  return ORBX_OK;
}

int orbx_debug_sincos(orbx_ctx* ctx, const float* angle_deg, int n, float* cos_out, float* sin_out) {
  if (!ctx || n < 0 || (n > 0 && (!angle_deg || !cos_out || !sin_out))) return ORBX_E_BADARG;
  if (n == 0) return ORBX_OK;
  if (hipSetDevice(ctx->device) != hipSuccess) return ORBX_E_HIP;
  DeviceBuf<float> d;
  HIPCHK(d.grow((size_t)n * 3 * sizeof(float)));
  HIPCHK(hipMemcpyAsync(d, angle_deg, (size_t)n * sizeof(float), hipMemcpyHostToDevice, ctx->st));
  HIPCHK(launch_debug_sincos(ctx->st, d, n, d + n, d + 2 * (size_t)n, ctx->libmVariant));
  HIPCHK(hipMemcpyAsync(cos_out, d + n, (size_t)n * sizeof(float), hipMemcpyDeviceToHost, ctx->st));
  HIPCHK(hipMemcpyAsync(sin_out, d + 2 * (size_t)n, (size_t)n * sizeof(float), hipMemcpyDeviceToHost, ctx->st));
  HIPCHK(hipStreamSynchronize(ctx->st));
  return ORBX_OK;
}

int orbx_debug_std_sort(orbx_ctx* ctx, int32_t* triples, int n) {
  if (!ctx || n < 0 || (n > 0 && !triples)) return ORBX_E_BADARG;
  if (n == 0) return ORBX_OK;
  if (hipSetDevice(ctx->device) != hipSuccess) return ORBX_E_HIP;
  DeviceBuf<int> d;
  DeviceBuf<unsigned long long> w;
  HIPCHK(d.grow((size_t)n * 3 * sizeof(int)));
  HIPCHK(w.grow((size_t)n * 2 * sizeof(unsigned long long)));
  HIPCHK(hipMemcpyAsync(d, triples, (size_t)n * 3 * sizeof(int), hipMemcpyHostToDevice, ctx->st));
  HIPCHK(launch_debug_sort(ctx->st, d, n, w, w + n));
  HIPCHK(hipMemcpyAsync(triples, d, (size_t)n * 3 * sizeof(int), hipMemcpyDeviceToHost, ctx->st));
  HIPCHK(hipStreamSynchronize(ctx->st));
  return ORBX_OK;
}

}

namespace orbx {
int ctxDevice(const orbx_ctx* c) { return c->device; }
hipStream_t ctxStream(const orbx_ctx* c) { return c->st; }
int ctxDrain(orbx_ctx* c) {
  if (hipSetDevice(c->device) != hipSuccess) return ORBX_E_HIP;
  return waitAll(c);
}
void ctxSetError(orbx_ctx* c, const char* msg) { c->err = msg; }
DeviceBuf<uint8_t>& ctxIo(orbx_ctx* c) { return c->io; }
InitScratch* ctxInit(orbx_ctx* c) { return &c->init; }
MatchBowScratch* ctxMatchBow(orbx_ctx* c) { return &c->matchBow; }
BaScratch* ctxBa(orbx_ctx* c) { return &c->ba; }
PoseScratch* ctxPose(orbx_ctx* c) { return &c->pose; }
PnpScratch* ctxPnp(orbx_ctx* c) { return &c->pnp; }
Sim3Scratch* ctxSim3(orbx_ctx* c) { return &c->sim3; }
Sim3OptScratch* ctxSim3Opt(orbx_ctx* c) { return &c->sim3Opt; }
LbaScratch* ctxLba(orbx_ctx* c) { return &c->lba; }
MapScratch* ctxMap(orbx_ctx* c) { return &c->map; }
TriScratch* ctxTri(orbx_ctx* c) { return &c->tri; }
const float* ctxInvSigma2(const orbx_ctx* c, int* nlevels) {
  *nlevels = c->p.nlevels;
  return c->invSigma2.data();
}
const float* ctxSigma2(const orbx_ctx* c, int* nlevels) {
  *nlevels = c->p.nlevels;
  return c->sigma2.data();
}
const float* ctxScale(const orbx_ctx* c, int* nlevels) {
  *nlevels = c->p.nlevels;
  return c->scale.data();
}
}
```

### orb_slam_tracking_amd/csrc/orbx_device.h

```cpp
#pragma once
#include <algorithm>
#include <cstdint>

#include "../../include/orbx.h"

#define ORBX_MAX_LEVELS 16
#define ORBX_EDGE 19
#define ORBX_MIN_BORDER 16
#define ORBX_CELL_MAX 76
#define ORBX_GRID_COLS 64
#define ORBX_GRID_ROWS 48

namespace orbx {

struct LevelGeom {
  int32_t w, h, stride;
  int32_t nCols, nRows;
  int32_t wCell, hCell;
  int32_t maxBX, maxBY;
  int32_t cellBase;
  int32_t candCap;
  int32_t quota;
  int32_t xtabOff, ytabOff;
  int32_t patchSize;
  float scale;
  int64_t imgOff;
  int64_t frameStride;
  int64_t candOff;
  int32_t resizeSpanOk;
  uint32_t colsInv24;
  int32_t segCap;
  int32_t candMax;
};

struct Geom {
  int32_t nlevels;
  int32_t nCellsTotal;
  int32_t iniTh, minTh;
  int32_t selCap;
  int32_t frame0;
  LevelGeom L[ORBX_MAX_LEVELS];
};

struct FastCell {
  uint32_t imgOff;
  uint32_t segOff;
  uint32_t stride;
  uint32_t nw_ch;
  uint32_t iw_ih;
  uint32_t xoff_level;
  uint32_t ox_oy;
  uint32_t segCap;
};
static_assert(sizeof(FastCell) == 32, "FastCell is loaded with one s_load_dwordx8");

#if defined(__HIPCC__)
#define ORBX_HD __host__ __device__
#else
#define ORBX_HD
#endif
ORBX_HD static inline uint32_t packCand(int x, int y, int score) { return (uint32_t)x | ((uint32_t)y << 12) | ((uint32_t)score << 24); }

struct SelKp {
  uint16_t x, y;
  uint8_t level, response;
  uint16_t pad;
};

struct OctLevel {
  int32_t width, height;
  int32_t nIni;
  float hX;
  int32_t wCell, hCell, nCols;
  int32_t quota;
  int32_t cellBase, nCells, segCap;
  int32_t depthBits;
  int32_t tabOff, tabW, tabH;
  int32_t bigD0, bigBuckets, bigCapB;
  int32_t bigDMax;
  int32_t bigTabOff;
};
#define ORBX_OCTB_CAP 1024
#define ORBX_OCTB_MAX_BUCKETS 1024
#define ORBX_OCTB_INFO 40

struct DescStage {
  const SelKp* selStage;
  const int* nselLevel;
  int* nsel;
  int* nselUser;
  int* hostNsel;
  int* hostErr;
  int* maxN;
  int* hostMaxN;
  int32_t selStride;
  int32_t selOff[ORBX_MAX_LEVELS];
};
#define ORBX_DESC_STAGED_MAX_UNITS 256

struct OctLaunch {
  OctLevel lev[ORBX_MAX_LEVELS];
  int64_t candOff[ORBX_MAX_LEVELS];
  int64_t scrOff[ORBX_MAX_LEVELS];
  int64_t scrStride[ORBX_MAX_LEVELS];
  int32_t candCap[ORBX_MAX_LEVELS];
  int32_t selOff[ORBX_MAX_LEVELS];
  int32_t scrNMax[ORBX_MAX_LEVELS];
  int32_t nlevels, selStride;
  int32_t frame0, nCellsTotal;
  const uint32_t* codeTab;
};

#define ORBX_OCT_MAX_CAND ((1 << 19) - 1)
#define ORBX_OCT_FEEDBACK(n, fill, depth) ((int)(n) | ((((int)(fill) + 3) >> 2) << 19) | ((int)(depth) << 28))
#define ORBX_OCT_FB_COUNT(v) ((int)(v) & 0x7ffff)
#define ORBX_OCT_FB_FILL(v) ((((int)(v) >> 19) & 0x1ff) << 2)
#define ORBX_OCT_FB_DEPTH(v) (((int)(v) >> 28) & 7)
#define ORBX_OCT_FB_MAXF(a, b, F) (F(a) > F(b) ? F(a) : F(b))
#define ORBX_OCT_FB_MAX(a, b) ORBX_OCT_FEEDBACK(ORBX_OCT_FB_MAXF(a, b, ORBX_OCT_FB_COUNT), ORBX_OCT_FB_MAXF(a, b, ORBX_OCT_FB_FILL), ORBX_OCT_FB_MAXF(a, b, ORBX_OCT_FB_DEPTH))
#define ORBX_OCT_REDONE 0x40000000

#if defined(__HIPCC__)
__device__ __forceinline__ int selUnitCount(int raw, bool* failed) {
  *failed = *failed || raw < 0;
  return raw < 0 ? 0 : (raw & ~ORBX_OCT_REDONE);
}
__device__ __forceinline__ void selPublishFrame(int f, int total, bool failed, int* __restrict__ nsel, int* __restrict__ nselUser,
                                                int* __restrict__ hostNsel, int* __restrict__ hostErr) {
  nsel[f] = total;
  if (nselUser) nselUser[f] = total;
  if (hostNsel) hostNsel[f] = total;
  if (failed) *hostErr = 1;
}
__device__ __forceinline__ void selReduceReports(int lane, int frame0, int nFrames, int nlevels, int* __restrict__ maxN,
                                                 int* __restrict__ hostMaxN) {
  static_assert(ORBX_MAX_LEVELS <= 16, "sixteen lanes per frame");
  int m = 0;
  if ((lane & 15) < nlevels)
    for (int fr = lane >> 4; fr < nFrames; fr += 4) {
      const int idx = (frame0 + fr) * nlevels + (lane & 15);
      const int v = maxN[idx];
      m = ORBX_OCT_FB_MAX(m, v);
      maxN[idx] = 0;
    }
  { const int t = __shfl_xor(m, 16); m = ORBX_OCT_FB_MAX(m, t); }
  { const int t = __shfl_xor(m, 32); m = ORBX_OCT_FB_MAX(m, t); }
  if (lane < nlevels) hostMaxN[lane] = m;
}
#endif


inline void octBigChoose(OctLevel* O, int nMax, int hint, int fillPrev = 0, int dPrev = 0, int* estFill = nullptr) {
  O->bigD0 = 0; O->bigBuckets = 0; O->bigCapB = 0;
  if (estFill) *estFill = 0;
  if (O->bigDMax < 0) return;
  int d = 0;
  if (hint > 0) {
    while (d < O->bigDMax && (long long)hint > 256ll * ((long long)O->nIni << (2 * d))) d++;
  } else {
    const double rootArea = (double)(O->width / O->nIni + 1) * (double)O->height;
    while (d < O->bigDMax && rootArea / (double)(1ll << (2 * d)) > 16384.0) d++;
  }
  long long nPad = 1024;
  while (nPad < nMax) nPad <<= 1;
  auto capOf = [&](int dd) {
    const long long nb = (long long)O->nIni << (2 * dd);
    int cap = ORBX_OCTB_CAP;
    while (cap > 0 && (long long)cap * nb > nPad) cap >>= 1;
    return cap;
  };
  auto bound = [&](int dd) -> long long {
    if (fillPrev <= 0) return 0;
    return dd <= dPrev ? (long long)fillPrev << (2 * (dPrev - dd)) : (long long)fillPrev;
  };
  while (d < O->bigDMax && bound(d) * 4 > 3ll * capOf(d)) d++;
  const long long nb = (long long)O->nIni << (2 * d);
  const int cap = capOf(d);
  if (cap < 256 || nb > ORBX_OCTB_MAX_BUCKETS) return;
  O->bigD0 = d; O->bigBuckets = (int32_t)nb; O->bigCapB = cap;
  if (estFill) *estFill = (int)std::min<long long>(bound(d), 1 << 20);
}

struct CopySeg {
  const uint32_t* src;
  uint32_t* dst;
  const int32_t* cnt;
  int32_t rows, rowDwords, mult, pad;
};
struct CopyOut {
  CopySeg s[6];
};

struct ResizeTab {
  int32_t ofs;
  int32_t coef;
};

struct PyrTileRect {
  int16_t nx0, nx1, ny0, ny1;
  int16_t ox0, ox1, oy0, oy1;
};
struct PyrTileTap {
  uint32_t pos;
  uint32_t coef;
};
#define ORBX_PYR_TILE_TAPS 768

// ... 643 lines not shown
```

### orb_slam_tracking_amd/csrc/orbx_kernels.hip

```cpp
#include <hip/hip_runtime.h>

#include <algorithm>
#include <cstdint>
#include <cstdio>
#include <cstdlib>
#include <type_traits>

#include "../../include/orbx.h"
#include "orbx_launch.h"
#include "orbx_knobs.h"

namespace orbx {

__global__ __launch_bounds__(256) void k_resize(const uint8_t* __restrict__ src, long long srcFrameStride, int sw, int sh,
                                                int sstride, uint8_t* __restrict__ dst, long long dstFrameStride, int dw,
                                                int dh, int dstride, const ResizeTab* __restrict__ xtab,
                                                const ResizeTab* __restrict__ ytab) {
  const int f = blockIdx.z;
  const int dx0 = (blockIdx.x * 64 + threadIdx.x) * 4;
  const int dy = blockIdx.y * 4 + threadIdx.y;
  if (dx0 >= dw || dy >= dh) return;
  const ResizeTab ty = ytab[dy];
  const int sy0 = min(max(ty.ofs, 0), sh - 1), sy1 = min(max(ty.ofs + 1, 0), sh - 1);
  const int b0 = ty.coef & 0xffff, b1 = ty.coef >> 16;
// ... 383 lines not shown
    R = k == 0 ? __builtin_elementwise_maximum(a0, a1) : __builtin_elementwise_maximum(__builtin_elementwise_maximum(R, a0), a1);
  }
  const uint32_t r = __builtin_bit_cast(uint32_t, R);
  return max(r & 0xffffu, r >> 16);
}

__global__ __launch_bounds__(FAST_T) void k_fast(const uint8_t* __restrict__ img0, long long img0FrameStride, int img0Aligned,
                                              const uint8_t* __restrict__ pyr, const Geom g,
                                              uint32_t* __restrict__ cand, int* __restrict__ cellCount,
                                              const FastLds fl) {
  extern __shared__ __attribute__((aligned(16))) uint8_t fastLds[];
  uint8_t* const tile = fastLds;
  uint8_t* const smap = fastLds + fl.tileBytes;
  uint16_t* const list = reinterpret_cast<uint16_t*>(fastLds + fl.tileBytes + fl.smapBytes);
  uint32_t* const outl = reinterpret_cast<uint32_t*>(fastLds + fl.tileBytes + fl.smapBytes + fl.listBytes);
  __shared__ int nList, nOut;

  const int t = threadIdx.x;
  const int f = blockIdx.y + g.frame0;
  int level = 0;
  const int cid = blockIdx.x;
  while (level + 1 < g.nlevels && cid >= g.L[level + 1].cellBase) level++;
  const LevelGeom& L = g.L[level];
  const int local = cid - L.cellBase;
  const int ci = (int)(((uint32_t)local * L.colsInv24) >> 24), cj = local - ci * L.nCols;
  const int iniY = ORBX_MIN_BORDER + ci * L.hCell;
  const int iniX = ORBX_MIN_BORDER + cj * L.wCell;
  int* const myCount = cellCount + (long long)f * g.nCellsTotal + cid;
  if (iniY >= L.maxBY - 3 || iniX >= L.maxBX - 6) {
    if (t == 0) *myCount = 0;
    return;
  }
  const int maxY = min(iniY + L.hCell + 6, L.maxBY), maxX = min(iniX + L.wCell + 6, L.maxBX);
  const int cw = maxX - iniX, ch = maxY - iniY;
  if (cw < 7 || ch < 7) {
    if (t == 0) *myCount = 0;
    return;
  }
  const int iw = cw - 6, ih = ch - 6;

  const uint8_t* base;
  int stride;
  bool aligned = true;
  if (level == 0) {
    base = img0 + (long long)f * img0FrameStride;
    stride = L.stride;
    aligned = img0Aligned != 0;
  } else {
    base = pyr + L.imgOff + (long long)f * L.frameStride;
    stride = L.stride;
  }
  const int ax0 = aligned ? (iniX & ~3) : iniX;
  const int xoff = iniX - ax0;
  if (aligned) {
    const int nw = (maxX - ax0 + 3) >> 2;
    const uint32_t invNw = c_inv20.v[nw];
    uint32_t* tile32 = reinterpret_cast<uint32_t*>(tile);
    const int r0 = (int)(((uint32_t)t * invNw) >> 20), c0 = t - r0 * nw;
    const int dr = (int)(((uint32_t)FAST_T * invNw) >> 20), dc = FAST_T - dr * nw;
    uint32_t goff = (uint32_t)((iniY + r0) * stride + ax0 + 4 * c0);
    const uint32_t dGoff = (uint32_t)(dr * stride + 4 * dc), wrapG = (uint32_t)(stride - 4 * nw);
    int lidx = r0 * (TILE_STRIDE / 4) + c0, c = c0;
    const int dLidx = dr * (TILE_STRIDE / 4) + dc, wrapL = TILE_STRIDE / 4 - nw;
#pragma unroll 1
    for (int idx = t; idx < nw * ch; idx += FAST_T) {
      tile32[lidx] = *reinterpret_cast<const uint32_t*>(base + goff);
      c += dc; goff += dGoff; lidx += dLidx;
      if (c >= nw) { c -= nw; goff += wrapG; lidx += wrapL; }
    }
  } else {
    const uint32_t invCw = c_inv20.v[cw];
    for (int idx = t; idx < cw * ch; idx += FAST_T) {
      const int r = (int)(((uint32_t)idx * invCw) >> 20), c = idx - r * cw;
      tile[r * TILE_STRIDE + c] = base[(long long)(iniY + r) * stride + iniX + c];
    }
  }
  {
    uint4* smap128 = reinterpret_cast<uint4*>(smap);
    for (int idx = t; idx < fl.smapBytes / 16; idx += FAST_T) smap128[idx] = make_uint4(0u, 0u, 0u, 0u);
  }
  if (t == 0) { nList = 0; nOut = 0; }
  __syncthreads();

  constexpr int RS = TILE_STRIDE;
  constexpr int ro[16] = {3 * RS,      3 * RS + 1,  2 * RS + 2,  RS + 3,  3,       -RS + 3,     -2 * RS + 2, -3 * RS + 1,
                          -3 * RS,     -3 * RS - 1, -2 * RS - 2, -RS - 3, -3,      RS - 3,      2 * RS - 2,  3 * RS - 1};
  const int py0 = (int)(((uint32_t)t * c_inv20.v[iw]) >> 20), px0 = t - py0 * iw;
  const int dpy = (int)(((uint32_t)FAST_T * c_inv20.v[iw]) >> 20), dpx = FAST_T - dpy * iw;
  const int npix = iw * ih;
  const int off0 = (py0 + 3) * TILE_STRIDE + xoff + px0 + 3, dOff = dpy * TILE_STRIDE + dpx;
  for (int pass = 0; pass < 2; pass++) {
    const int th = pass == 0 ? g.iniTh : g.minTh;
    {
      int px = px0, off = off0;
      for (int idx = t; idx < npix; idx += FAST_T) {
        const uint8_t* p = &tile[off];
        const int v = p[0], hi = v + th, lo = v - th;
        const int q0 = p[ro[0]], q4 = p[ro[4]], q8 = p[ro[8]], q12 = p[ro[12]];
        const bool b0 = q0 > hi, b4 = q4 > hi, b8 = q8 > hi, b12 = q12 > hi;
        const bool d0 = q0 < lo, d4 = q4 < lo, d8 = q8 < lo, d12 = q12 < lo;
        const bool cand0 = ((b0 | b8) & (b4 | b12)) | ((d0 | d8) & (d4 | d12));
        if (cand0) list[atomicAdd(&nList, 1)] = (uint16_t)off;
        px += dpx;
        off += dOff;
        if (px >= iw) { px -= iw; off += TILE_STRIDE - iw; }
      }
    }
    __syncthreads();
    const int nl = nList;
    for (int e = t; e < nl; e += FAST_T) {
      const int off = list[e];
      const uint8_t* p = &tile[off];
      uint32_t q[16];
#pragma unroll
      for (int k = 0; k < 16; k++) q[k] = p[ro[k]];
      const int s = (int)fastStrengthBiased(p[0], q) - (int)FAST_PK_BIAS;
      if (s > th) {
        const int row = (off * 3121) >> 18;
        smap[(row - 2) * SMAP_STRIDE + (off - row * TILE_STRIDE - xoff - 2)] = (uint8_t)s;
      } else {
        list[e] = 0xFFFF;
      }
    }
    __syncthreads();
    for (int e = t; e < nl; e += FAST_T) {
      const int off = list[e];
      if (off == 0xFFFF) continue;
      const int row = (off * 3121) >> 18;
      const int py = row - 3, px = off - row * TILE_STRIDE - xoff - 3;
      const uint8_t* q = &smap[(py + 1) * SMAP_STRIDE + px + 1];
      const int s = q[0];
      const int n0 = q[-SMAP_STRIDE - 1], n1 = q[-SMAP_STRIDE], n2 = q[-SMAP_STRIDE + 1], n3 = q[-1], n4 = q[1],
                n5 = q[SMAP_STRIDE - 1], n6 = q[SMAP_STRIDE], n7 = q[SMAP_STRIDE + 1];
      const int nmax = max(max(max(n0, n1), max(n2, n3)), max(max(n4, n5), max(n6, n7)));
      const bool keep = s > 1 && s > nmax;
      if (keep) {
        const int slot = atomicAdd(&nOut, 1);
        if (slot < fl.outCap) outl[slot] = packCand(px + 3 + cj * L.wCell, py + 3 + ci * L.hCell, s - 1);
      }
    }
    __syncthreads();
    if (nOut > 0 || pass == 1 || g.minTh >= g.iniTh) break;
    if (t == 0) nList = 0;
    __syncthreads();
  }
  const int no = min(nOut, fl.outCap);
  if (t == 0) *myCount = no;
  if (no > 0) {
    uint32_t* dstc = cand + L.candOff + (long long)f * L.candCap + (long long)local * L.segCap;
    for (int e = t; e < no; e += FAST_T) dstc[e] = outl[e];
  }
}

#define FW_RING 192
#define FW_CORN 256
#define FW_CPW 1
#define FW_XK 16

__device__ __forceinline__ int fwMbcnt(unsigned long long m) {
  return (int)__builtin_amdgcn_mbcnt_hi((uint32_t)(m >> 32), __builtin_amdgcn_mbcnt_lo((uint32_t)m, 0u));
}

typedef __attribute__((address_space(3))) uint8_t fw_lds_u8;
typedef __attribute__((address_space(3))) uint16_t fw_lds_u16;
typedef __attribute__((address_space(3))) uint32_t fw_lds_u32;
__device__ __forceinline__ const fw_lds_u8* fwLds8(const uint32_t a) { return reinterpret_cast<const fw_lds_u8*>((size_t)a); }
__device__ __forceinline__ const fw_lds_u16* fwLds16(const uint32_t a) { return reinterpret_cast<const fw_lds_u16*>((size_t)a); }
__device__ __forceinline__ const fw_lds_u32* fwLds32(const uint32_t a) { return reinterpret_cast<const fw_lds_u32*>((size_t)a); }
__device__ __forceinline__ void fwStoreB16(const uint32_t addr, const uint32_t val, const unsigned long long m) {
  unsigned long long saved;
  asm volatile("s_mov_b64 %0, exec\n\ts_mov_b64 exec, %1\n\tds_write_b16 %2, %3\n\ts_mov_b64 exec, %0"
               : "=&s"(saved)
               : "s"(m), "v"(addr), "v"(val)
               : "memory");
}
__device__ __forceinline__ void fwStoreB8(const uint32_t addr, const uint32_t val, const unsigned long long m) {
  unsigned long long saved;
  asm volatile("s_mov_b64 %0, exec\n\ts_mov_b64 exec, %1\n\tds_write_b8 %2, %3\n\ts_mov_b64 exec, %0"
               : "=&s"(saved)
               : "s"(m), "v"(addr), "v"(val)
               : "memory");
}
__device__ __forceinline__ unsigned long long fwGtLo(const uint32_t x, const uint32_t thLo) {
  unsigned long long m;
  asm("v_cmp_lt_i16_e64 %0, %1, %2" : "=s"(m) : "s"(thLo), "v"(x));
  return m;
}
__device__ __forceinline__ unsigned long long fwGtHi(const uint32_t x, const uint32_t thHi) {
  unsigned long long m;
  asm("v_cmp_lt_i32_e64 %0, %1, %2" : "=s"(m) : "s"(thHi), "v"(x));
  return m;
}

template <int TS>
__device__ __forceinline__ uint32_t fwStrength(const uint32_t e) {
  constexpr int C = 3 * TS + 3;
  constexpr int ro[16] = {C + 3 * TS,  C + 3 * TS + 1, C + 2 * TS + 2, C + TS + 3, C + 3,  C - TS + 3, C - 2 * TS + 2, C - 3 * TS + 1,
                          C - 3 * TS,  C - 3 * TS - 1, C - 2 * TS - 2, C - TS - 3, C - 3,  C + TS - 3, C + 2 * TS - 2, C + 3 * TS - 1};
  const fw_lds_u8* const p = fwLds8(e);
  uint32_t q[16];
#pragma unroll
  for (int k = 0; k < 16; k++) q[k] = p[ro[k]];
  return fastStrengthBiased(p[C], q);
}

typedef short short2v __attribute__((ext_vector_type(2)));

template <int TS>
__global__ __launch_bounds__(64) void k_fast_wave(const uint8_t* __restrict__ img0, long long img0FrameStride,
                                                  const uint8_t* __restrict__ pyr, const Geom g,
                                                  const FastCell* __restrict__ cells, uint32_t* __restrict__ cand,
                                                  int* __restrict__ cellCount, const int tileBytes, const int smapBytes) {
  extern __shared__ __attribute__((aligned(16))) uint8_t fwLds[];
  const int lane = threadIdx.x;
  uint8_t* const tile = fwLds + 16;
  uint8_t* const smap = tile + tileBytes;
  const uint32_t ldsBase = (uint32_t)(size_t)(fw_lds_u8*)fwLds;
  const uint32_t tileAddr = ldsBase + 16u, smapAddr = tileAddr + (uint32_t)tileBytes;
  const uint32_t ringAddr = smapAddr + (uint32_t)smapBytes, cornAddr = ringAddr + 2u * FW_RING;
  const uint32_t ringLane = ringAddr + 2u * (uint32_t)lane;
  const int nGroups = (g.nCellsTotal + FW_CPW - 1) / FW_CPW;
  const int xq = (int)((blockIdx.x + blockIdx.y) & 7u), xi = (int)(blockIdx.x >> 3);
  const int grp = ((xi / FW_XK) * 8 + xq) * FW_XK + (xi % FW_XK);
  if (grp >= nGroups) return;
  const int f = blockIdx.y + g.frame0;
  const int cid0 = (nGroups - 1 - grp) * FW_CPW, cid1 = min(cid0 + FW_CPW, g.nCellsTotal);
  for (int cid = cid0; cid < cid1; cid++) {
  const FastCell c = cells[cid];
  int* const myCount = cellCount + (long long)f * g.nCellsTotal + cid;
  const int ch = (int)(c.nw_ch >> 16);
  if (ch == 0) {
    if (lane == 0) *myCount = 0;
    continue;
  }
  const int level = (int)(c.xoff_level >> 16);
  const LevelGeom& L = g.L[level];
  const uint8_t* const base =
      (level == 0 ? img0 + (long long)f * img0FrameStride : pyr + L.imgOff + (long long)f * L.frameStride) + c.imgOff;
  {
    typedef uint32_t u32x4_a4 __attribute__((ext_vector_type(4), aligned(4)));
    constexpr int NQ = TS / 16;
    const int stride = (int)c.stride;
    if (lane < ch) {
      const uint8_t* p = base + (unsigned)(lane * stride);
      u32x4_a4 q[NQ];
#pragma unroll
      for (int j = 0; j < NQ; j++) q[j] = *reinterpret_cast<const u32x4_a4*>(p + 16 * j);
      uint4* const dst = reinterpret_cast<uint4*>(tile + lane * TS);
#pragma unroll
      for (int j = 0; j < NQ; j++) dst[j] = make_uint4(q[j].x, q[j].y, q[j].z, q[j].w);
    }
  }
  const int iw = (int)(c.iw_ih & 0xffffu), ih = (int)(c.iw_ih >> 16), xoff = (int)(c.xoff_level & 0xffffu);
  const int ox = (int)(int16_t)(c.ox_oy & 0xffffu), oy = (int)(c.ox_oy >> 16);
  {
    uint4* const s128 = reinterpret_cast<uint4*>(smap);
    for (int i = lane; i < (ih + 2) * (TS / 16); i += 64) s128[i] = make_uint4(0u, 0u, 0u, 0u);
  }
  __builtin_amdgcn_wave_barrier();

  constexpr int RS = TS;
  const uint32_t kN = smapAddr - tileAddr - (uint32_t)xoff, kS = kN + (uint32_t)(TS + 1);
  const uint32_t eIdle = tileAddr + (uint32_t)xoff;
  const int nqc = (iw + 3) >> 2, nItems = nqc * ih;
  const uint32_t inv = c_inv20.v[nqc];
  const int qy0 = (int)(((uint32_t)lane * inv) >> 20), qc0 = lane - qy0 * nqc;
  const int dqy = (int)((64u * inv) >> 20), dqc = 64 - dqy * nqc;
  const int sh = (xoff + 3) & 3;
  const uint32_t pos0 = ((uint32_t)qc0 << 16) | (tileAddr + (uint32_t)(qy0 * TS + xoff + 3 - sh + 4 * qc0 - 4));
  const uint32_t dPos = ((uint32_t)dqc << 16) | (uint32_t)(dqy * TS + 4 * dqc);
  const uint32_t wrapK = (uint32_t)(TS - 4 * nqc) - ((uint32_t)nqc << 16);
  const uint32_t lastThr = (uint32_t)(nqc - 1) << 16;
  const int nvLast = iw - 4 * (nqc - 1);
  const uint32_t aLast = tileAddr + (uint32_t)((ih - 1) * TS + xoff + 3 - sh + 4 * (nqc - 1) - 4);
  const uint32_t selC0 = 0x0c000c00u + (uint32_t)sh * 0x00010001u + 0x00010000u, selC1 = selC0 + 0x00020002u;
  const uint32_t selL0 = selC0 + 0x00010001u, selL1 = selL0 + 0x00020002u;
  const bool rNear = sh <= 1;
  const uint32_t rOff4 = rNear ? 0u : 4u;
  const uint32_t selR0 = 0x0c000c00u + (uint32_t)(rNear ? sh + 3 : sh - 1) * 0x00010001u + 0x00010000u, selR1 = selR0 + 0x00020002u;
  uint32_t* const dstc = cand + L.candOff + (long long)f * L.candCap + c.segOff;
  const int segCap = (int)c.segCap;
  int nOut = 0;
  for (int pass = 0; pass < 2; pass++) {
    const int th = pass == 0 ? g.iniTh : g.minTh;
    const uint32_t thLo = (uint32_t)th, thHi = ((uint32_t)th << 16) | 0xffffu;
    const int thB = th + (int)FAST_PK_BIAS;
    int nList = 0, nCorn = 0;
    bool flat = pass == 0;
    short2v looseMax = {-0x8000, -0x8000};
    auto flush = [&](const int cnt) {
      __builtin_amdgcn_wave_barrier();
      const int keepN = nList - cnt;
      uint32_t e = (uint32_t)fwLds16(ringLane)[keepN];
      unsigned long long act = ~0ull;
      if (cnt < 64) {
        asm volatile("" ::: "memory");
        act = (1ull << cnt) - 1ull;
        e = lane < cnt ? e : eIdle;
      }
      const uint32_t sv = fwStrength<TS>(e);
      const unsigned long long mc = __ballot((int)sv > thB) & act;
      if (mc != 0ull) {
        fwStoreB8(e + kS, sv, mc);
        const int nc = (int)__popcll(mc);
        if (nCorn + nc <= FW_CORN) fwStoreB16((cornAddr + 2u * (uint32_t)nCorn) + 2u * (uint32_t)fwMbcnt(mc), e, mc);
        nCorn += nc;
      }
      nList = keepN;
    };
    {
      uint32_t pos = pos0;
      for (int idx0 = 0; idx0 < nItems; idx0 += 64) {
        uint32_t a = pos & 0xffffu;
        const bool tail = idx0 + 64 > nItems;
        if (tail) {
          asm volatile("" ::: "memory");
          a = min(a, aLast);
        }
        const fw_lds_u32* const pa = fwLds32(a);
        const uint32_t t0 = pa[1], t1 = pa[2];
        const uint32_t cM = pa[3 * (TS / 4)], c0 = pa[3 * (TS / 4) + 1], c1 = pa[3 * (TS / 4) + 2];
        const uint32_t b0 = pa[6 * (TS / 4) + 1], b1 = pa[6 * (TS / 4) + 2];
        const fw_lds_u32* const pr = fwLds32(a + rOff4);
        const uint32_t rlo = pr[3 * (TS / 4) + 1], rhi = pr[3 * (TS / 4) + 2];
        short2v d[2];
#pragma unroll
        for (int hp = 0; hp < 2; hp++) {
          const uint32_t V = __builtin_amdgcn_perm(c1, c0, hp ? selC1 : selC0);
          const uint32_t QL = __builtin_amdgcn_perm(c0, cM, hp ? selL1 : selL0), QR = __builtin_amdgcn_perm(rhi, rlo, hp ? selR1 : selR0);
          const uint32_t QT = __builtin_amdgcn_perm(t1, t0, hp ? selC1 : selC0), QB = __builtin_amdgcn_perm(b1, b0, hp ? selC1 : selC0);
          const ushort2v vV = __builtin_bit_cast(ushort2v, V), vL = __builtin_bit_cast(ushort2v, QL), vR = __builtin_bit_cast(ushort2v, QR),
                         vT = __builtin_bit_cast(ushort2v, QT), vB = __builtin_bit_cast(ushort2v, QB);
          const ushort2v mx = __builtin_elementwise_min(__builtin_elementwise_max(vT, vB), __builtin_elementwise_max(vL, vR));
          const ushort2v mn = __builtin_elementwise_max(__builtin_elementwise_min(vT, vB), __builtin_elementwise_min(vL, vR));
          d[hp] = __builtin_elementwise_max(__builtin_bit_cast(short2v, mx) - __builtin_bit_cast(short2v, vV),
                                            __builtin_bit_cast(short2v, vV) - __builtin_bit_cast(short2v, mn));
        }
        const uint32_t dm = __builtin_bit_cast(uint32_t, __builtin_elementwise_max(d[0], d[1]));
        if (flat) {
          asm volatile("" ::: "memory");
          looseMax = __builtin_elementwise_max(looseMax, __builtin_bit_cast(short2v, dm));
        }
        if ((fwGtLo(dm, thLo) | fwGtHi(dm, thHi)) != 0ull) {
          flat = false;
          unsigned long long keepEnd = ~0ull;
          if (nvLast < 4) keepEnd = ~__ballot(pos >= lastThr);
          const unsigned long long live = tail ? (1ull << (nItems - idx0)) - 1ull : ~0ull;
          const uint32_t q0 = a + (uint32_t)(sh + 1);
#pragma unroll
          for (int j = 0; j < 4; j++) {
            const uint32_t dj = __builtin_bit_cast(uint32_t, d[j >> 1]);
            unsigned long long m = ((j & 1) ? fwGtHi(dj, thHi) : fwGtLo(dj, thLo)) & live;
            if (j >= nvLast) m &= keepEnd;
            if (m != 0ull) {
              fwStoreB16((ringAddr + 2u * (uint32_t)nList) + 2u * (uint32_t)fwMbcnt(m), q0 + (uint32_t)j, m);
              nList += (int)__popcll(m);
            }
            if (j & 1)
              while (nList >= 64) flush(64);
          }
        }
        pos += dPos;
        pos = min(pos, pos + wrapK);
      }
      if (nList > 0) flush(nList);
    }
    __builtin_amdgcn_wave_barrier();
    auto nms = [&](const uint32_t eIn, const bool act) {
      const uint32_t e = act ? eIn : eIdle;
      const fw_lds_u8* const q = fwLds8(e + kN);
      const int sv = q[RS + 1];
      const int n0 = q[0], n1 = q[1], n2 = q[2], n3 = q[RS], n4 = q[RS + 2], n5 = q[2 * RS], n6 = q[2 * RS + 1], n7 = q[2 * RS + 2];
      const int nmax = max(max(max(n0, n1), max(n2, n3)), max(max(n4, n5), max(n6, n7)));
      const bool keep = act && sv > 1 && sv > nmax;
      const unsigned long long mk = __ballot(keep);
      if (keep) {
        const int slot = nOut + fwMbcnt(mk);
        const int o = (int)(e - tileAddr) + 3 * TS + 3;
        const int row = TS == 64 ? (o >> 6) : (int)(((uint32_t)o * 43691u) >> 21);
        static_assert(TS == 64 || TS == 48, "row split of a tile offset");
        if (slot < segCap) dstc[slot] = packCand(o - row * TS + ox, row + oy, sv - 1);
      }
      nOut += (int)__popcll(mk);
    };
    if (nCorn <= FW_CORN) {
      for (int e0 = 0; e0 < nCorn; e0 += 64) nms((uint32_t)fwLds16(cornAddr)[min(e0 + lane, FW_CORN - 1)], e0 + lane < nCorn);
    } else {
      const uint32_t invw = c_inv20.v[iw];
      const int py0 = (int)(((uint32_t)lane * invw) >> 20), px0 = lane - py0 * iw;
      const int dpy = (int)((64u * invw) >> 20), dpx = 64 - dpy * iw;
      int px = px0;
      uint32_t e = eIdle + (uint32_t)(py0 * TS + px0);
      const int npix = iw * ih;
      for (int idx0 = 0; idx0 < npix; idx0 += 64) {
        const bool live = idx0 + lane < npix;
        const int sv = live ? (int)fwLds8(e + kS)[0] : 0;
        const unsigned long long any = __ballot(sv > 0);
        if (any) nms(e, sv > 0);
        px += dpx;
        e += (uint32_t)(dpy * TS + dpx);
        if (px >= iw) { px -= iw; e += (uint32_t)(TS - iw); }
      }
    }
    if (nOut > 0 || pass == 1 || g.minTh >= g.iniTh) break;
    {
      const uint32_t lm = __builtin_bit_cast(uint32_t, looseMax);
      if (flat && (fwGtLo(lm, (uint32_t)g.minTh) | fwGtHi(lm, ((uint32_t)g.minTh << 16) | 0xffffu)) == 0ull) break;
    }
  }
  if (lane == 0) *myCount = min(nOut, segCap);
  __builtin_amdgcn_wave_barrier();
  }
}

constexpr int8_t k_pattern[256 * 4] = {
#include "orbx_pattern_data.inc"
};
struct PatternF {
  float v[256 * 4];
};
constexpr PatternF makePatternF() {
  PatternF t{};
  for (int i = 0; i < 256 * 4; i++) t.v[i] = (float)k_pattern[i];
  return t;
}
__device__ const PatternF d_patternf = makePatternF();
__constant__ int c_umax[16] = {15, 15, 15, 15, 14, 14, 14, 13, 13, 12, 11, 10, 9, 8, 6, 3};

__device__ __forceinline__ int reflect101(int p, int n) {
  if (p < 0) p = -p;
  if (p >= n) p = 2 * n - 2 - p;
  return p;
}

#include "orbx_sincos_tab.inc"
template <bool UNIFORM>
__device__ __forceinline__ void sincosTable(double x, double* sn, double* cs) {
  const double k = rint(x * ORBX_128OPI);
  double r = fma(-k, ORBX_PIO128_HI, x);
  r = fma(-k, ORBX_PIO128_LO, r);
  int ki = (int)k & 255;
  if (UNIFORM) ki = __builtin_amdgcn_readfirstlane(ki);
  const double sk = d_sincosTab[ki][0], ck = d_sincosTab[ki][1];
  const double z = r * r;
  const double ps = fma(z, fma(z, -1.0 / 5040.0, 1.0 / 120.0), -1.0 / 6.0);
  const double pc = fma(z, fma(z, -1.0 / 720.0, 1.0 / 24.0), -0.5);
  const double sr = fma(z * r, ps, r), cm1 = z * pc;
  *sn = fma(ck, sr, fma(sk, cm1, sk));
  *cs = fma(-sk, sr, fma(ck, cm1, ck));
}

__device__ __forceinline__ void sincosfGlibc(float y, float* sn, float* cs) {
  const double x = (double)y;
  const double r = x * 0x1.45F306DC9C883p+23;
  const int n = ((int)r + 0x800000) >> 24;
  const double xr = fma(-(double)n, 0x1.921FB54442D18p0, x);
  const double sg = ((n ^ (n >> 1)) & 1) ? -1.0 : 1.0;
  const double xs = xr * sg, x2 = xr * xr;
  const double x3 = xs * x2, s1 = fma(x2, -0x1.994eb3774cf24p-13, 0x1.1107605230bc4p-7), x7 = x3 * x2;
  const double S = fma(x7, s1, fma(x3, -0x1.555545995a603p-3, xs));
  const double x4 = x2 * x2, c2 = fma(x2, 0x1.99343027bf8c3p-16, -0x1.6c087e89a359dp-10);
  const double c1 = fma(x2, -0x1.ffffffd0c621cp-2, 0x1p0), x6 = x4 * x2;
  const double C0 = fma(x6, c2, fma(x4, 0x1.55553e1068f19p-5, c1));
  const float Sf = (float)S, C0f = (float)C0;
  const float Cf = (n & 2) ? -C0f : C0f;
  *sn = (n & 1) ? Cf : Sf;
  *cs = (n & 1) ? Sf : Cf;
}

__device__ __forceinline__ float fast_atan2_deg(float y, float x) {
  const float p1 = 0.9997878412794807f * (float)(180 / 3.14159265358979323846);
  const float p3 = -0.3258083974640975f * (float)(180 / 3.14159265358979323846);
  const float p5 = 0.1555786518463281f * (float)(180 / 3.14159265358979323846);
  const float p7 = -0.04432655554792128f * (float)(180 / 3.14159265358979323846);
  const float eps = (float)2.2204460492503131e-16;
  const float ax = fabsf(x), ay = fabsf(y);
  float a, c, c2;
  if (ax >= ay) {
    c = ay / (ax + eps);
    c2 = c * c;
    a = (((p7 * c2 + p5) * c2 + p3) * c2 + p1) * c;
  } else {
    c = ax / (ay + eps);
    c2 = c * c;
    a = 90.f - (((p7 * c2 + p5) * c2 + p3) * c2 + p1) * c;
  }
  if (x < 0) a = 180.f - a;
  if (y < 0) a = 360.f - a;
  return a;
}


#define PW_ROWS 43
#define PW_WORDS 13
#define PW_ROWS_PAD 48
#define BL_STRIDE 48
#define BL_COLS 48
#define PW_RAW_WORDS (PW_ROWS_PAD * PW_WORDS)
#define PW_WAVE_WORDS (PW_RAW_WORDS + 4)

struct IcTables {
  uint32_t w1[16 * 8], wu[16 * 8];
};
constexpr IcTables makeIcTables() {
  IcTables t{};
  constexpr int um[16] = {15, 15, 15, 15, 14, 14, 14, 13, 13, 12, 11, 10, 9, 8, 6, 3};
  for (int av = 0; av < 16; av++)
    for (int j = 0; j < 8; j++) {
      uint32_t m1 = 0, mu = 0;
      for (int b = 0; b < 4; b++) {
        const int u = -15 + 4 * j + b, au = u < 0 ? -u : u;
        if (au <= um[av]) {
          m1 |= 1u << (8 * b);
          mu |= (uint32_t)(u + 15) << (8 * b);
        }
      }
      t.w1[av * 8 + j] = m1;
      t.wu[av * 8 + j] = mu;
    }
  return t;
}
__device__ const IcTables d_ic = makeIcTables();

#define DESC_WAVES 3
#define DESC_PAIR_WAVES 3
constexpr int descWaves(const int kpw) { return kpw == 2 ? DESC_PAIR_WAVES : DESC_WAVES; }

static_assert(32 + (10 - 3) > 36, "tile 2's swapped-tap product only touches columns / rows past the 37 x 37 patch");
struct BlurFrags {
  uint32_t w[4][64][2];
};
template <int GV>
constexpr int blurTap(int j) {
  const int T[7] = {18, 34, GV ? 49 : 48, GV ? 55 : 56, GV ? 49 : 48, 34, 18};
  return j >= 0 && j < 7 ? T[j] : 0;
}
template <int GV>
constexpr BlurFrags makeBlurFrags() {
  BlurFrags t{};
  for (int s = 0; s < 4; s++)
    for (int lane = 0; lane < 64; lane++)
      for (int e = 0; e < 2; e++)
        for (int b = 0; b < 4; b++)
          t.w[s][lane][e] |= (uint32_t)blurTap<GV>(16 * e + 4 * (lane >> 4) - (lane & 15) - s + b) << (8 * b);
  return t;
}
constexpr int blurFragByte(const BlurFrags& t, int s, int tile, int lane, int d, int b) {
  return d == tile ? (int)(t.w[s][lane][0] >> (8 * b) & 0xff) : d == tile + 1 ? (int)(t.w[s][lane][1] >> (8 * b) & 0xff) : 0;
}
template <int GV>
constexpr bool blurFragsOk() {
  const BlurFrags t = makeBlurFrags<GV>();
  for (int s = 0; s < 4; s++)
    for (int c = 0; c < BL_COLS; c++) {
      int sum = 0;
      for (int q = 0; q < 4; q++)
        for (int d = 0; d < 4; d++)
          for (int b = 0; b < 4; b++) {
            const int v = blurFragByte(t, s, c >> 4, (c & 15) + 16 * q, d, b);
            if (v > 127 || v != blurTap<GV>(16 * d + 4 * q + b - s - c)) return false;
            sum += v;
          }
      if (c < 37 && sum != (GV ? 257 : 256)) return false;
// ... 1689 lines not shown
                                                 int h, int c0, int c1, int c2, int shift, int srcAligned, uint8_t* __restrict__ dst,
                                                 long long dstFrameStride, int dstride, int dstAligned) {
  const uint32_t half = 1u << (shift - 1);
  const int x = (blockIdx.x * 256 + threadIdx.x) * 4;
  const int y = blockIdx.y;
  if (x >= w) return;
  const uint8_t* s = src + (size_t)blockIdx.z * srcFrameStride + (size_t)y * sstride + (size_t)3 * x;
  uint8_t* d = dst + (size_t)blockIdx.z * dstFrameStride + (size_t)y * dstride + x;
  uint32_t out = 0;
  if (x + 4 <= w && srcAligned) {
    const uint32_t* s4 = reinterpret_cast<const uint32_t*>(s);
    const uint32_t a = s4[0], b = s4[1], c = s4[2];
    const uint32_t y0 = ((a & 255) * c0 + ((a >> 8) & 255) * c1 + ((a >> 16) & 255) * c2 + half) >> shift;
    const uint32_t y1 = ((a >> 24) * c0 + (b & 255) * c1 + ((b >> 8) & 255) * c2 + half) >> shift;
    const uint32_t y2 = (((b >> 16) & 255) * c0 + (b >> 24) * c1 + (c & 255) * c2 + half) >> shift;
    const uint32_t y3 = (((c >> 8) & 255) * c0 + ((c >> 16) & 255) * c1 + (c >> 24) * c2 + half) >> shift;
    out = y0 | y1 << 8 | y2 << 16 | y3 << 24;
    if (dstAligned) {
      *reinterpret_cast<uint32_t*>(d) = out;
      return;
    }
    d[0] = (uint8_t)y0; d[1] = (uint8_t)y1; d[2] = (uint8_t)y2; d[3] = (uint8_t)y3;
    return;
  }
  const int n = min(4, w - x);
  for (int i = 0; i < n; i++) d[i] = (uint8_t)((s[3 * i] * c0 + s[3 * i + 1] * c1 + s[3 * i + 2] * c2 + half) >> shift);
}

__global__ __launch_bounds__(256) void k_copy_rows(const uint8_t* __restrict__ src, long long srcFrameStride, int sstride, int w,
                                                   int h, uint8_t* __restrict__ dst, long long dstFrameStride, int dstride) {
  const int x = blockIdx.x * 256 + threadIdx.x;
  if (x >= w) return;
  dst[(size_t)blockIdx.z * dstFrameStride + (size_t)blockIdx.y * dstride + x] =
      src[(size_t)blockIdx.z * srcFrameStride + (size_t)blockIdx.y * sstride + x];
}

hipError_t launch_to_gray(hipStream_t st, int nFrames, const uint8_t* src, long long srcFrameStride, int sstride, int w, int h,
                          int channels, int rgb, uint8_t* dst, long long dstFrameStride, int dstride, int grayVariant) {
  if (nFrames <= 0) return hipSuccess;
  if (channels == 1) {
    dim3 block(256, 1, 1), grid((w + 255) / 256, h, nFrames);
    hipLaunchKernelGGL(k_copy_rows, grid, block, 0, st, src, srcFrameStride, sstride, w, h, dst, dstFrameStride, dstride);
    return hipGetLastError();
  }
  const int srcAligned = ((uintptr_t)src % 4 == 0) && (srcFrameStride % 4 == 0) && (sstride % 4 == 0);
  const int dstAligned = ((uintptr_t)dst % 4 == 0) && (dstFrameStride % 4 == 0) && (dstride % 4 == 0);
  dim3 block(256, 1, 1), grid((w + 1023) / 1024, h, nFrames);
  const int cr = grayVariant ? 9798 : 4899, cg = grayVariant ? 19235 : 9617, cb = grayVariant ? 3735 : 1868, shift = grayVariant ? 15 : 14;
  hipLaunchKernelGGL(k_to_gray, grid, block, 0, st, src, srcFrameStride, sstride, w, h, rgb ? cr : cb, cg, rgb ? cb : cr, shift,
                     srcAligned, dst, dstFrameStride, dstride, dstAligned);
  return hipGetLastError();
}

__global__ __launch_bounds__(256) void k_copy_out(const CopyOut c) {
  const CopySeg& s = c.s[blockIdx.z];
  for (int row = blockIdx.y; row < s.rows; row += gridDim.y) {
    const int n = s.cnt ? min(max(s.cnt[row], 0) * s.mult, s.rowDwords) : s.rowDwords;
    const uint32_t* src = s.src + (long long)row * s.rowDwords;
    uint32_t* dst = s.dst + (long long)row * s.rowDwords;
    for (int i = blockIdx.x * 256 + threadIdx.x; i < n; i += gridDim.x * 256) dst[i] = src[i];
  }
}
hipError_t launch_copy_out(hipStream_t st, const CopyOut& c, int nseg, int maxRows) {
  if (nseg <= 0) return hipSuccess;
  hipLaunchKernelGGL(k_copy_out, dim3(8, (unsigned)std::min(std::max(maxRows, 1), 1024), (unsigned)nseg), dim3(256), 0, st, c);
  return hipGetLastError();
}

__global__ __launch_bounds__(256) void k_debug_sincos(const float* __restrict__ angle, int n, float* __restrict__ c, float* __restrict__ s,
                                                      const int libmFloat) {
  const int i = blockIdx.x * 256 + threadIdx.x;
  if (i >= n) return;
  const float factorPI = (float)(3.14159265358979323846 / 180.f);
  if (libmFloat) {
    sincosfGlibc(angle[i] * factorPI, &s[i], &c[i]);
    return;
  }
  double sd, cd;
  sincosTable<false>((double)(angle[i] * factorPI), &sd, &cd);
  c[i] = (float)cd;
  s[i] = (float)sd;
}
hipError_t launch_debug_sincos(hipStream_t st, const float* angle, int n, float* c, float* s, int libmFloat) {
  if (n <= 0) return hipSuccess;
  hipLaunchKernelGGL(k_debug_sincos, dim3((n + 255) / 256), dim3(256), 0, st, angle, n, c, s, libmFloat);
  return hipGetLastError();
}

hipError_t launch_check_model(hipStream_t st, int nModels, const ScoreArgs& a) {
  if (nModels <= 0) return hipSuccess;
  hipLaunchKernelGGL(k_check_model, dim3(nModels), dim3(64), 0, st, a);
  return hipGetLastError();
}

hipError_t launch_undistort(hipStream_t st, int nFrames, const orbx_keypoint* in, const int* nkp, int capacity, const CamD& c,
                            orbx_keypoint* out) {
  if (nFrames <= 0 || capacity <= 0) return hipSuccess;
  dim3 block(256, 1, 1), grid((capacity + 255) / 256, nFrames, 1);
  hipLaunchKernelGGL(k_undistort, grid, block, 0, st, in, nkp, capacity, c, out);
  return hipGetLastError();
}

hipError_t launch_pyramid_tiles(hipStream_t st, int nFrames, const uint8_t* img0, long long img0FrameStride, uint8_t* pyr,
                                const Geom& g, const PyrTileRect* rects, const PyrTileTap* taps, int nTiles, int buf0Bytes,
                                int bufBytes) {
  const size_t lds = ORBX_PYR_TILE_TAPS * sizeof(PyrTileTap) + (size_t)buf0Bytes + 2 * (size_t)bufBytes;
  hipLaunchKernelGGL(k_pyramid_tiles, dim3(nTiles, nFrames, 1), dim3(256, 1, 1), lds, st, img0, img0FrameStride, pyr, g, rects, taps,
                     buf0Bytes, bufBytes);
  return hipGetLastError();
}

hipError_t launch_resize(hipStream_t st, int nFrames, const uint8_t* src, long long srcFrameStride, int sw, int sh, int sstride,
                         uint8_t* dst, long long dstFrameStride, int dw, int dh, int dstride, const ResizeTab* xtab,
                         const ResizeTab* ytab, int dwordPath, int wideFrames) {
  dim3 block(64, 4, 1), grid((dw + 255) / 256, (dh + 3) / 4, nFrames);
  if (dwordPath)
    hipLaunchKernelGGL(k_resize_dw, dim3(grid.x, (dh + 4 * RESIZE_DW_ROWS - 1) / (4 * RESIZE_DW_ROWS), nFrames), block, 0, st, src, srcFrameStride, sw, sh, sstride, dst, dstFrameStride, dw, dh,
                       dstride, xtab, ytab, wideFrames);
  else
    hipLaunchKernelGGL(k_resize, grid, block, 0, st, src, srcFrameStride, sw, sh, sstride, dst, dstFrameStride, dw, dh, dstride,
                       xtab, ytab);
  return hipGetLastError();
}

hipError_t launch_pyramid_bands(hipStream_t st, int nFrames, const uint8_t* img0, long long img0FrameStride, uint8_t* pyr,
                                const Geom& g, const ResizeTab* tab, const PyrBands& pb) {
  if (nFrames <= 0 || g.nlevels <= 1) return hipSuccess;
  dim3 block(PYR_T, 1, 1), grid(pb.nBands * pb.nStrips, nFrames, 1);
  if (pb.maxRows > 256 || pb.maxRows < 1 || pb.nStrips < 1 || pb.nStrips > ORBX_PYR_STRIPS_MAX) return hipErrorInvalidValue;
  const bool one = !pb.twoGroups;
  const size_t lds = 2 * ((size_t)pb.maxRows + 1) * sizeof(uint4);
  const uint4* tab4 = reinterpret_cast<const uint4*>(tab);
  if (pb.dual2 && one) hipLaunchKernelGGL((k_pyramid_bands<1, 1>), grid, block, lds, st, img0, img0FrameStride, pyr, g, tab4, pb);
  else if (pb.dual2) hipLaunchKernelGGL((k_pyramid_bands<1, 2>), grid, block, lds, st, img0, img0FrameStride, pyr, g, tab4, pb);
  else if (one) hipLaunchKernelGGL((k_pyramid_bands<0, 1>), grid, block, lds, st, img0, img0FrameStride, pyr, g, tab4, pb);
  else hipLaunchKernelGGL((k_pyramid_bands<0, 2>), grid, block, lds, st, img0, img0FrameStride, pyr, g, tab4, pb);
  return hipGetLastError();
}

hipError_t launch_fast(hipStream_t st, int nFrames, const uint8_t* img0, long long img0FrameStride, int img0Aligned,
                       const uint8_t* pyr, const Geom& g, uint32_t* cand, int* cellCount, const FastCell* cells, int waveOk,
                       int* usedWave) {
  int cw = 7, ch = 7;
  for (int l = 0; l < g.nlevels; l++) {
    cw = std::max(cw, std::min(g.L[l].wCell + 6, ORBX_CELL_MAX));
    ch = std::max(ch, std::min(g.L[l].hCell + 6, ORBX_CELL_MAX));
  }
  const int wgMaxCells = (int)knob(KNOB_FAST_WG_MAX_CELLS, 5000);
  const bool small = (long long)nFrames * g.nCellsTotal <= wgMaxCells;
  if (usedWave) *usedWave = (waveOk && img0Aligned && cells && !small) ? 1 : 0;
  if (waveOk && img0Aligned && cells && !small) {
    const int groups = ((g.nCellsTotal + FW_CPW - 1) / FW_CPW + 8 * FW_XK - 1) / (8 * FW_XK) * (8 * FW_XK);
    const int ts = waveOk == 2 ? 48 : 64;
    const int tileBytes = ch * ts + 16, smapBytes = (ch - 6 + 2) * ts;
    const size_t lds = (size_t)(16 + tileBytes + smapBytes + FW_RING * 2 + FW_CORN * 2);
    if (ts == 48)
      hipLaunchKernelGGL(k_fast_wave<48>, dim3(groups, nFrames, 1), dim3(64, 1, 1), lds, st, img0, img0FrameStride, pyr, g, cells,
                         cand, cellCount, tileBytes, smapBytes);
    else
      hipLaunchKernelGGL(k_fast_wave<64>, dim3(groups, nFrames, 1), dim3(64, 1, 1), lds, st, img0, img0FrameStride, pyr, g, cells,
                         cand, cellCount, tileBytes, smapBytes);
    return hipGetLastError();
  }
  dim3 block(FAST_T, 1, 1), grid(g.nCellsTotal, nFrames, 1);
  FastLds fl;
  fl.tileBytes = (ch * TILE_STRIDE + 15) & ~15;
  fl.smapBytes = (SMAP_STRIDE * (ch - 6 + 2) + 15) & ~15;
  fl.listBytes = (2 * (cw - 6) * (ch - 6) + 15) & ~15;
  fl.outCap = ((cw - 6 + 1) / 2) * ((ch - 6 + 1) / 2);
  const size_t lds = (size_t)fl.tileBytes + fl.smapBytes + fl.listBytes + (size_t)fl.outCap * 4;
  hipLaunchKernelGGL(k_fast, grid, block, lds, st, img0, img0FrameStride, img0Aligned, pyr, g, cand, cellCount, fl);
  return hipGetLastError();
}

hipError_t launch_describe_patch(hipStream_t st, int nFrames, int maxSel, const uint8_t* img0, long long img0FrameStride,
                                 int img0Aligned, const uint8_t* pyr, const Geom& g, const SelKp* sel, const int* nsel,
                                 orbx_keypoint* kps, uint8_t* desc, int capacity, int gaussVariant, int libmFloat,
                                 const DescStage* staged) {
  if (maxSel <= 0 && !staged) return hipSuccess;
  const int perGroup = staged ? DESC_WAVES : 2 * DESC_PAIR_WAVES;
  dim3 block(64 * (staged ? DESC_WAVES : DESC_PAIR_WAVES), 1, 1), grid(((maxSel + perGroup - 1) / perGroup + 7) / 8 * 8, nFrames, 1);
  const DescStage none = {};
  if (staged) {
    if (gaussVariant)
      hipLaunchKernelGGL((k_describe_patch<1, true>), grid, block, 0, st, img0, img0FrameStride, img0Aligned, pyr, g, sel, nsel, kps,
                         desc, capacity, *staged, libmFloat);
    else
      hipLaunchKernelGGL((k_describe_patch<0, true>), grid, block, 0, st, img0, img0FrameStride, img0Aligned, pyr, g, sel, nsel, kps,
                         desc, capacity, *staged, libmFloat);
  } else if (gaussVariant)
    hipLaunchKernelGGL((k_describe_patch<1, false, 2>), grid, block, 0, st, img0, img0FrameStride, img0Aligned, pyr, g, sel, nsel, kps,
                       desc, capacity, none, libmFloat);
  else
    hipLaunchKernelGGL((k_describe_patch<0, false, 2>), grid, block, 0, st, img0, img0FrameStride, img0Aligned, pyr, g, sel, nsel, kps,
                       desc, capacity, none, libmFloat);
  return hipGetLastError();
}

hipError_t launch_match(hipStream_t st, int nPairs, const int* dFirst, const int* dSecond, const orbx_keypoint* kps,
                        const uint8_t* desc, const int* nkp, int capacity, orbx_bounds b, int window, float nnratio, int checkOri,
                        int* matches12, int* nmatches, int* stats, int* scratch, int pair0, int wideMode, int* hostWide,
                        unsigned int* diag) {
  if (nPairs <= 0) return hipSuccess;
  MatchParams mp;
  mp.capacity = capacity; mp.window = window; mp.nnratio = nnratio; mp.checkOri = checkOri; mp.b = b;
  mp.noGeneral = knobOn(KNOB_MATCH_NO_GENERAL) ? 1 : 0;
  mp.noMfma = knobOn(KNOB_MATCH_NO_MFMA) ? 1 : 0;
  mp.pair0 = pair0;
  mp.dmax = TH_LOW + 1;
  while (mp.dmax < 257 && !(nnratio * (float)mp.dmax >= (float)TH_LOW)) mp.dmax++;
  const long long stride = matchScratchStride(capacity);
  const int capl = matchWideCap(capacity);
  const size_t lds = (size_t)capl * 12;
  if (wideMode != 2)
    hipLaunchKernelGGL((k_match_jacobi<256, 4, 16>), dim3(nPairs), dim3(1024), 0, st, dFirst, dSecond, kps, desc, nkp, mp,
                       matches12, nmatches, stats, scratch, stride, capl, hostWide);
  if (wideMode == 2)
    hipLaunchKernelGGL(k_match_wide_prep, dim3(nPairs), dim3(MW_T), 0, st, dFirst, dSecond, kps, nkp, mp, matches12, nmatches,
                       scratch, stride, capl);
  if (wideMode != 0) {
    const long long w2 = 2ll * window, ex = b.max_x - b.min_x, ey = b.max_y - b.min_y;
    const bool bfPossible = (long long)nPairs * ((capl + 255) >> 8) >= 256 && w2 * ORBX_GRID_COLS > (ORBX_GRID_COLS - 3) * ex &&
                            w2 * ORBX_GRID_ROWS > (ORBX_GRID_ROWS - 3) * ey;
    if (!mp.noMfma && bfPossible)
      hipLaunchKernelGGL(k_match_bf_mfma, dim3((capl + BF_QWG - 1) / BF_QWG, nPairs), dim3(BF_T), 0, st, dFirst, dSecond, kps, desc, nkp, mp,
                         nmatches, scratch, scratch, stride, capl, diag);
    {
      const long long wgs = (long long)nPairs * ((capl + 63) / 64);
      if (wgs <= 512)
        hipLaunchKernelGGL(k_match_wide_lists<8>, dim3((capl + 63) / 64, nPairs), dim3(512), 0, st, dFirst, dSecond, kps, desc, nkp, mp,
                           nmatches, scratch, scratch, stride, capl);
      else
        hipLaunchKernelGGL(k_match_wide_lists<4>, dim3((capl + 63) / 64, nPairs), dim3(256), 0, st, dFirst, dSecond, kps, desc, nkp, mp,
                           nmatches, scratch, scratch, stride, capl);
    }
    const int qpw = (long long)nPairs * capl >= 100000 ? 16 : 4;
    hipLaunchKernelGGL(k_match_wide_sort, dim3((capl + 4 * qpw - 1) / (4 * qpw), nPairs), dim3(256), 0, st, mp, nmatches, scratch, stride,
                       capl, qpw);
    hipLaunchKernelGGL(k_match_wide_resolve, dim3(nPairs), dim3(MW_T), lds, st, dFirst, dSecond, kps, desc, nkp, mp, matches12,
                       nmatches, stats, scratch, stride, capl);
  }
  return hipGetLastError();
}

}
```

Before: 531,100.

## Precompute FAST wave per-cell constants on host into 64-byte cell records

Moves per-cell derived constants (divisor reciprocals, position steps, select masks, tail counts, LDS addresses, absolute image/candidate offsets) from the k_fast_wave kernel into host-built 64-byte FastCell records, loaded with one s_load_dwordx16. The kernel loop is split into full and last steps via templated lambdas, and ring/corner counters become LDS address tops. Exec-mask save/restore in the inline-asm stores is dropped in favour of restoring exec to -1. This trims scalar ALU work and per-cell setup, at the cost of larger records and reliance on full exec at every store site. A debug entry point for dumping the cell records is added.

```diff
diff --git a/include/orbx.h b/include/orbx.h
--- a/include/orbx.h
+++ b/include/orbx.h
@@ -783,6 +783,8 @@
 
 int orbx_debug_last_launch(const orbx_ctx* ctx, int32_t* info8);
 int orbx_debug_pyr_cols(int groups, int two_groups, uint32_t* info5);
+int orbx_debug_fast_cells(const orbx_params* params, int width, int height, int stride0, int max_batch, uint32_t* records, int cap,
+                          int32_t* info4);
 int orbx_debug_match_counters(orbx_ctx* ctx, uint32_t* info4);
 int orbx_debug_set(const char* key, long long value);
 int orbx_debug_path_codes(int width, int height, int n, const int32_t* xs, const int32_t* ys, uint64_t* from_tables,
diff --git a/orb_slam_tracking_amd/__init__.py b/orb_slam_tracking_amd/__init__.py
--- a/orb_slam_tracking_amd/__init__.py
+++ b/orb_slam_tracking_amd/__init__.py
@@ -307,6 +307,7 @@
     L.orbx_debug_set.argtypes = [ctypes.c_char_p, ctypes.c_longlong]
     L.orbx_debug_last_launch.argtypes = [vp, vp]
     L.orbx_debug_pyr_cols.argtypes = [ctypes.c_int, ctypes.c_int, vp]
+    L.orbx_debug_fast_cells.argtypes = [vp, ctypes.c_int, ctypes.c_int, ctypes.c_int, ctypes.c_int, vp, ctypes.c_int, vp]
     L.orbx_debug_match_counters.argtypes = [vp, vp]
     L.orbx_debug_selection_units.argtypes = [vp, i32, vp, vp]
     L.orbx_debug_path_codes.argtypes = [ctypes.c_int, ctypes.c_int, ctypes.c_int, vp, vp, vp, vp]
diff --git a/orb_slam_tracking_amd/csrc/orbx_api.cpp b/orb_slam_tracking_amd/csrc/orbx_api.cpp
--- a/orb_slam_tracking_amd/csrc/orbx_api.cpp
+++ b/orb_slam_tracking_amd/csrc/orbx_api.cpp
@@ -76,18 +76,23 @@
   }
 };
 
-struct orbx_ctx {
+struct ExtractorSetup {
   orbx_params p{};
+  int maxB = 0;
+  std::vector<float> scale, invScale, sigma2, invSigma2;
+  std::vector<int> quota;
+  int umax[16]{};
+  int libmVariant = ORBX_LIBM_DEFAULT;
+  int selCap = 0;
+  std::string err;
+};
+
+struct orbx_ctx : ExtractorSetup {
   int device = 0;
   hipStream_t st = nullptr;
   bool ownStream = false;
-  int maxW = 0, maxH = 0, maxB = 0;
-  std::vector<float> scale, invScale, sigma2, invSigma2;
-  std::vector<int> quota;
-  int umax[16]{};
+  int maxW = 0, maxH = 0;
   int gaussVariant = 0, grayVariant = 0;
-  int libmVariant = ORBX_LIBM_DEFAULT;
-  int selCap = 0;
 
   int curW = 0, curH = 0, curStride0 = 0;
   Geom g{};
@@ -180,13 +185,11 @@
   int parity = 0;
   double ms[ORBX_STAGE_COUNT]{};
   int64_t launches[ORBX_STAGE_COUNT]{};
-
-  std::string err;
 };
 
 namespace {
 
-void computeTables(orbx_ctx* c) {
+void computeTables(ExtractorSetup* c) {
   const int nl = c->p.nlevels;
   const double scaleFactor = (double)c->p.scale_factor;
   c->scale.assign(nl, 1.f);
@@ -227,7 +230,7 @@
   }
 }
 
-void levelSize(const orbx_ctx* c, int w, int h, int l, int* lw, int* lh) {
+void levelSize(const ExtractorSetup* c, int w, int h, int l, int* lw, int* lh) {
   *lw = cvRoundF(w * c->invScale[l]);
   *lh = cvRoundF(h * c->invScale[l]);
 }
@@ -290,7 +293,7 @@
   }
 }
 
-int buildGeometry(orbx_ctx* c, int w, int h, int stride0, Geom* out, std::vector<ResizeTab>* tab, PyrTabInfo* pyrInfo = nullptr) {
+int buildGeometry(ExtractorSetup* c, int w, int h, int stride0, Geom* out, std::vector<ResizeTab>* tab, PyrTabInfo* pyrInfo = nullptr) {
   Geom g{};
   g.nlevels = c->p.nlevels;
   g.iniTh = std::min(std::max(c->p.ini_th_fast, 0), 255);
@@ -397,33 +400,70 @@
 
 int buildFastCells(const Geom& g, std::vector<FastCell>* out) {
   out->assign((size_t)g.nCellsTotal, FastCell{});
+  struct Rect {
+    int iniX, iniY, cw, ch;
+  };
+  auto rectOf = [](const LevelGeom& L, int ci, int cj) {
+    Rect r{ORBX_MIN_BORDER + cj * L.wCell, ORBX_MIN_BORDER + ci * L.hCell, 0, 0};
+    if (r.iniY >= L.maxBY - 3 || r.iniX >= L.maxBX - 6) return r;
+    const int maxY = std::min(r.iniY + L.hCell + 6, L.maxBY), maxX = std::min(r.iniX + L.wCell + 6, L.maxBX);
+    if (maxX - r.iniX < 7 || maxY - r.iniY < 7) return r;
+    r.cw = maxX - r.iniX;
+    r.ch = maxY - r.iniY;
+    return r;
+  };
   bool ok = true, narrow = true;
+  for (int l = 0; l < g.nlevels; l++) {
+    const LevelGeom& L = g.L[l];
+    if (L.segCap >= 2048 || L.candCap >= (1 << 30) || (l > 0 && (L.frameStride <= 0 || L.frameStride >= (int64_t)1 << 32))) ok = false;
+    for (int ci = 0; ci < L.nRows; ci++)
+      for (int cj = 0; cj < L.nCols; cj++) {
+        const Rect r = rectOf(L, ci, cj);
+        if (r.ch == 0) continue;
+        const int nw = (r.iniX + r.cw - (r.iniX & ~3) + 3) >> 2;
+        if (nw > 16 || r.ch > 64) ok = false;
+        if (nw > 12) narrow = false;
+      }
+  }
+  if (!ok) return 0;
+  const int TS = narrow ? 48 : 64;
+  const FastWaveLds lds = fastWaveLds(g, TS);
+  const uint32_t tileAddr = 16u;
   for (int l = 0; l < g.nlevels; l++) {
     const LevelGeom& L = g.L[l];
     for (int ci = 0; ci < L.nRows; ci++)
       for (int cj = 0; cj < L.nCols; cj++) {
+        const Rect r = rectOf(L, ci, cj);
+        if (r.ch == 0) continue;
         const int local = ci * L.nCols + cj;
         FastCell& c = (*out)[(size_t)L.cellBase + local];
-        c.xoff_level = (uint32_t)l << 16;
+        const int ax0 = r.iniX & ~3, xoff = r.iniX - ax0, iw = r.cw - 6, ih = r.ch - 6;
+        c.img = (uint64_t)(l == 0 ? 0 : L.imgOff) + (uint64_t)r.iniY * (uint64_t)L.stride + (uint64_t)ax0;
+        c.frameStride = l == 0 ? 0u : (uint32_t)L.frameStride;
         c.stride = (uint32_t)L.stride;
-        c.segOff = (uint32_t)local * (uint32_t)L.segCap;
-        c.segCap = (uint32_t)L.segCap;
-        const int iniY = ORBX_MIN_BORDER + ci * L.hCell, iniX = ORBX_MIN_BORDER + cj * L.wCell;
-        if (iniY >= L.maxBY - 3 || iniX >= L.maxBX - 6) continue;
-        const int maxY = std::min(iniY + L.hCell + 6, L.maxBY), maxX = std::min(iniX + L.wCell + 6, L.maxBX);
-        const int cw = maxX - iniX, ch = maxY - iniY;
-        if (cw < 7 || ch < 7) continue;
-        const int ax0 = iniX & ~3, xoff = iniX - ax0, nw = (maxX - ax0 + 3) >> 2;
-        if (nw > 16 || ch > 64) ok = false;
-        if (nw > 12) narrow = false;
-        c.imgOff = (uint32_t)(iniY * L.stride + ax0);
-        c.nw_ch = (uint32_t)nw | ((uint32_t)ch << 16);
-        c.iw_ih = (uint32_t)(cw - 6) | ((uint32_t)(ch - 6) << 16);
-        c.xoff_level |= (uint32_t)xoff;
-        c.ox_oy = ((uint32_t)(cj * L.wCell - xoff) & 0xffffu) | ((uint32_t)(ci * L.hCell) << 16);
+        c.cand = 4u * ((uint64_t)L.candOff + (uint64_t)local * (uint64_t)L.segCap);
+        c.candCap = 4u * (uint32_t)L.candCap;
+        c.oxy = (uint32_t)(cj * L.wCell - xoff) + ((uint32_t)(ci * L.hCell) << 12);
+        const int nqc = (iw + 3) >> 2, sh = (xoff + 3) & 3;
+        const uint32_t inv = ((1u << 20) + (uint32_t)nqc - 1u) / (uint32_t)nqc;
+        const int dqy = (int)((64u * inv) >> 20), dqc = 64 - dqy * nqc;
+        c.dPos = ((uint32_t)dqc << 16) | (uint32_t)(dqy * TS + 4 * dqc);
+        c.wrapK = (uint32_t)(TS - 4 * nqc) - ((uint32_t)nqc << 16);
+        c.selC0 = 0x0c000c00u + (uint32_t)sh * 0x00010001u + 0x00010000u;
+        c.selR0 = 0x0c000c00u + (uint32_t)(sh <= 1 ? sh + 3 : sh - 1) * 0x00010001u + 0x00010000u;
+        c.lastThr = (uint32_t)(nqc - 1) << 16;
+        const uint32_t aLast = tileAddr + (uint32_t)((ih - 1) * TS + xoff + 3 - sh + 4 * (nqc - 1) - 4);
+        const uint32_t kN = (uint32_t)lds.tileBytes - (uint32_t)xoff;
+        c.aLast_kN = aLast | (kN << 16);
+        const int nvLast = iw - 4 * (nqc - 1);
+        const uint32_t inside = (uint32_t)(nvLast > 1) | ((uint32_t)(nvLast > 2) << 1) | ((uint32_t)(nvLast > 3) << 2);
+        c.quad = inv | ((uint32_t)nqc << 21) | (inside << 25) | ((uint32_t)(sh >= 2) << 28) | ((uint32_t)(sh + 1) << 29);
+        const int nItems = nqc * ih, nFull = (nItems - 1) >> 6, nTail = nItems - 64 * nFull;
+        c.counts = (uint32_t)nFull | ((uint32_t)(64 - nTail) << 4) | ((uint32_t)L.segCap << 10) | ((uint32_t)r.ch << 21) |
+                   ((uint32_t)xoff << 28);
       }
   }
-  return ok ? (narrow ? 2 : 1) : 0;
+  return narrow ? 2 : 1;
 }
 
 struct Sizes {
@@ -2241,6 +2281,32 @@
   return ORBX_OK;
 }
 
+int orbx_debug_fast_cells(const orbx_params* params, int width, int height, int stride0, int max_batch, uint32_t* records, int cap,
+                          int32_t* info4) {
+  if (!params || !info4 || cap < 0 || (cap > 0 && !records) || params->nlevels < 1 || params->nlevels > ORBX_MAX_LEVELS ||
+      params->nfeatures < 1 || !(params->scale_factor >= 1.0f) || (params->scale_factor == 1.0f && params->nlevels > 1) || width < 1 ||
+      height < 1 || stride0 < width || max_batch < 1)
+    return ORBX_E_BADARG;
+  ExtractorSetup tmp;
+  tmp.p = *params;
+  tmp.maxB = max_batch;
+  computeTables(&tmp);
+  Geom g;
+  const int r = buildGeometry(&tmp, width, height, stride0, &g, nullptr);
+  if (r != ORBX_OK) return r;
+  std::vector<FastCell> cells;
+  const int ok = buildFastCells(g, &cells);
+  const FastWaveLds lds = fastWaveLds(g, ok == 2 ? 48 : 64);
+  info4[0] = g.nCellsTotal;
+  info4[1] = ok;
+  info4[2] = ok ? lds.tileBytes : 0;
+  info4[3] = ok ? lds.total : 0;
+  static_assert(sizeof(FastCell) == 16 * sizeof(uint32_t), "a record is sixteen dwords");
+  const size_t n = std::min((size_t)cap, cells.size());
+  if (n) memcpy(records, cells.data(), n * sizeof(FastCell));
+  return ORBX_OK;
+}
+
 int orbx_debug_last_launch(const orbx_ctx* ctx, int32_t* info8) {
   if (!ctx || !info8) return ORBX_E_BADARG;
   for (int i = 0; i < 8; i++) info8[i] = ctx->lastLaunch[i];
diff --git a/orb_slam_tracking_amd/csrc/orbx_device.h b/orb_slam_tracking_amd/csrc/orbx_device.h
--- a/orb_slam_tracking_amd/csrc/orbx_device.h
+++ b/orb_slam_tracking_amd/csrc/orbx_device.h
@@ -43,16 +43,35 @@
 };
 
 struct FastCell {
-  uint32_t imgOff;
-  uint32_t segOff;
+  uint64_t img;
+  uint32_t frameStride;
   uint32_t stride;
-  uint32_t nw_ch;
-  uint32_t iw_ih;
-  uint32_t xoff_level;
-  uint32_t ox_oy;
-  uint32_t segCap;
-};
-static_assert(sizeof(FastCell) == 32, "FastCell is loaded with one s_load_dwordx8");
+  uint64_t cand;
+  uint32_t candCap;
+  uint32_t oxy;
+  uint32_t dPos;
+  uint32_t wrapK;
+  uint32_t selC0, selR0;
+  uint32_t lastThr;
+  uint32_t aLast_kN;
+  uint32_t quad;
+  uint32_t counts;
+};
+static_assert(sizeof(FastCell) == 64, "FastCell is loaded with one s_load_dwordx16");
+#define ORBX_FW_RING 192
+#define ORBX_FW_CORN 256
+struct FastWaveLds {
+  int32_t tileBytes, smapBytes, total;
+};
+static inline FastWaveLds fastWaveLds(const Geom& g, int ts) {
+  int ch = 7;
+  for (int l = 0; l < g.nlevels; l++) ch = std::max(ch, std::min(g.L[l].hCell + 6, ORBX_CELL_MAX));
+  FastWaveLds r;
+  r.tileBytes = ch * ts + 16;
+  r.smapBytes = (ch - 6 + 2) * ts;
+  r.total = 16 + r.tileBytes + r.smapBytes + ORBX_FW_RING * 2 + ORBX_FW_CORN * 2;
+  return r;
+}
 
 #if defined(__HIPCC__)
 #define ORBX_HD __host__ __device__
diff --git a/orb_slam_tracking_amd/csrc/orbx_kernels.hip b/orb_slam_tracking_amd/csrc/orbx_kernels.hip
--- a/orb_slam_tracking_amd/csrc/orbx_kernels.hip
+++ b/orb_slam_tracking_amd/csrc/orbx_kernels.hip
@@ -559,8 +559,8 @@
   }
 }
 
-#define FW_RING 192
-#define FW_CORN 256
+#define FW_RING ORBX_FW_RING
+#define FW_CORN ORBX_FW_CORN
 #define FW_CPW 1
 #define FW_XK 16
 
@@ -575,17 +575,13 @@
 __device__ __forceinline__ const fw_lds_u16* fwLds16(const uint32_t a) { return reinterpret_cast<const fw_lds_u16*>((size_t)a); }
 __device__ __forceinline__ const fw_lds_u32* fwLds32(const uint32_t a) { return reinterpret_cast<const fw_lds_u32*>((size_t)a); }
 __device__ __forceinline__ void fwStoreB16(const uint32_t addr, const uint32_t val, const unsigned long long m) {
-  unsigned long long saved;
-  asm volatile("s_mov_b64 %0, exec\n\ts_mov_b64 exec, %1\n\tds_write_b16 %2, %3\n\ts_mov_b64 exec, %0"
-               : "=&s"(saved)
-               : "s"(m), "v"(addr), "v"(val)
-               : "memory");
-}
+  asm volatile("s_mov_b64 exec, %0\n\tds_write_b16 %1, %2\n\ts_mov_b64 exec, -1" : : "s"(m), "v"(addr), "v"(val) : "memory");
+}
+template <int OFF>
 __device__ __forceinline__ void fwStoreB8(const uint32_t addr, const uint32_t val, const unsigned long long m) {
-  unsigned long long saved;
-  asm volatile("s_mov_b64 %0, exec\n\ts_mov_b64 exec, %1\n\tds_write_b8 %2, %3\n\ts_mov_b64 exec, %0"
-               : "=&s"(saved)
-               : "s"(m), "v"(addr), "v"(val)
+  asm volatile("s_mov_b64 exec, %0\n\tds_write_b8 %1, %2 offset:%3\n\ts_mov_b64 exec, -1"
+               :
+               : "s"(m), "v"(addr), "v"(val), "n"(OFF)
                : "memory");
 }
 __device__ __forceinline__ unsigned long long fwGtLo(const uint32_t x, const uint32_t thLo) {
@@ -625,25 +621,30 @@
   const uint32_t ldsBase = (uint32_t)(size_t)(fw_lds_u8*)fwLds;
   const uint32_t tileAddr = ldsBase + 16u, smapAddr = tileAddr + (uint32_t)tileBytes;
   const uint32_t ringAddr = smapAddr + (uint32_t)smapBytes, cornAddr = ringAddr + 2u * FW_RING;
-  const uint32_t ringLane = ringAddr + 2u * (uint32_t)lane;
   const int nGroups = (g.nCellsTotal + FW_CPW - 1) / FW_CPW;
   const int xq = (int)((blockIdx.x + blockIdx.y) & 7u), xi = (int)(blockIdx.x >> 3);
   const int grp = ((xi / FW_XK) * 8 + xq) * FW_XK + (xi % FW_XK);
   if (grp >= nGroups) return;
   const int f = blockIdx.y + g.frame0;
+  const uint32_t fu = (uint32_t)f;
   const int cid0 = (nGroups - 1 - grp) * FW_CPW, cid1 = min(cid0 + FW_CPW, g.nCellsTotal);
   for (int cid = cid0; cid < cid1; cid++) {
-  const FastCell c = cells[cid];
-  int* const myCount = cellCount + (long long)f * g.nCellsTotal + cid;
-  const int ch = (int)(c.nw_ch >> 16);
+  FastCell c;
+  {
+    typedef uint32_t u32x16 __attribute__((ext_vector_type(16)));
+    u32x16 r;
+    asm volatile("s_load_dwordx16 %0, %1, 0x0\n\ts_waitcnt lgkmcnt(0)" : "=&s"(r) : "s"(cells + cid) : "memory");
+    c = __builtin_bit_cast(FastCell, r);
+  }
+  auto myCount = [&]() { return cellCount + (long long)((uint64_t)fu * (uint32_t)g.nCellsTotal + (uint32_t)cid); };
+  const int ch = (int)((c.counts >> 21) & 0x7fu);
   if (ch == 0) {
-    if (lane == 0) *myCount = 0;
+    if (lane == 0) *myCount() = 0;
     continue;
   }
-  const int level = (int)(c.xoff_level >> 16);
-  const LevelGeom& L = g.L[level];
-  const uint8_t* const base =
-      (level == 0 ? img0 + (long long)f * img0FrameStride : pyr + L.imgOff + (long long)f * L.frameStride) + c.imgOff;
+  const bool level0 = c.frameStride == 0u;
+  const uint8_t* const base = (level0 ? img0 : pyr) + (long long)fu * (level0 ? img0FrameStride : (long long)c.frameStride) +
+                              (long long)c.img;
   {
     typedef uint32_t u32x4_a4 __attribute__((ext_vector_type(4), aligned(4)));
     constexpr int NQ = TS / 16;
@@ -658,72 +659,77 @@
       for (int j = 0; j < NQ; j++) dst[j] = make_uint4(q[j].x, q[j].y, q[j].z, q[j].w);
     }
   }
-  const int iw = (int)(c.iw_ih & 0xffffu), ih = (int)(c.iw_ih >> 16), xoff = (int)(c.xoff_level & 0xffffu);
-  const int ox = (int)(int16_t)(c.ox_oy & 0xffffu), oy = (int)(c.ox_oy >> 16);
   {
     uint4* const s128 = reinterpret_cast<uint4*>(smap);
-    for (int i = lane; i < (ih + 2) * (TS / 16); i += 64) s128[i] = make_uint4(0u, 0u, 0u, 0u);
+    for (int i = lane; i < (ch - 4) * (TS / 16); i += 64) s128[i] = make_uint4(0u, 0u, 0u, 0u);
   }
   __builtin_amdgcn_wave_barrier();
 
   constexpr int RS = TS;
-  const uint32_t kN = smapAddr - tileAddr - (uint32_t)xoff, kS = kN + (uint32_t)(TS + 1);
-  const uint32_t eIdle = tileAddr + (uint32_t)xoff;
-  const int nqc = (iw + 3) >> 2, nItems = nqc * ih;
-  const uint32_t inv = c_inv20.v[nqc];
+  const uint32_t kN = c.aLast_kN >> 16;
+  const uint32_t eIdle = tileAddr + ((c.counts >> 28) & 3u);
+  const int nqc = (int)((c.quad >> 21) & 15u);
+  const int nFull = (int)(c.counts & 15u);
+  const uint32_t tailShift = (c.counts >> 4) & 63u;
+  const uint32_t inv = c.quad & 0x1fffffu;
   const int qy0 = (int)(((uint32_t)lane * inv) >> 20), qc0 = lane - qy0 * nqc;
-  const int dqy = (int)((64u * inv) >> 20), dqc = 64 - dqy * nqc;
-  const int sh = (xoff + 3) & 3;
-  const uint32_t pos0 = ((uint32_t)qc0 << 16) | (tileAddr + (uint32_t)(qy0 * TS + xoff + 3 - sh + 4 * qc0 - 4));
-  const uint32_t dPos = ((uint32_t)dqc << 16) | (uint32_t)(dqy * TS + 4 * dqc);
-  const uint32_t wrapK = (uint32_t)(TS - 4 * nqc) - ((uint32_t)nqc << 16);
-  const uint32_t lastThr = (uint32_t)(nqc - 1) << 16;
-  const int nvLast = iw - 4 * (nqc - 1);
-  const uint32_t aLast = tileAddr + (uint32_t)((ih - 1) * TS + xoff + 3 - sh + 4 * (nqc - 1) - 4);
-  const uint32_t selC0 = 0x0c000c00u + (uint32_t)sh * 0x00010001u + 0x00010000u, selC1 = selC0 + 0x00020002u;
+  const uint32_t sh1 = c.quad >> 29;
+  const uint32_t pos0 = ((uint32_t)qc0 << 16) + ((eIdle - sh1) + (uint32_t)(qy0 * TS + 4 * qc0));
+  const uint32_t dPos = c.dPos;
+  const uint32_t wrapK = c.wrapK;
+  const uint32_t lastThr = c.lastThr;
+  const unsigned long long quad64 = (unsigned long long)c.quad;
+  unsigned long long keepJ[4];
+  keepJ[0] = ~0ull;
+  asm("s_bfe_i64 %0, %1, 0x10019" : "=s"(keepJ[1]) : "s"(quad64) : "scc");
+  asm("s_bfe_i64 %0, %1, 0x1001a" : "=s"(keepJ[2]) : "s"(quad64) : "scc");
+  asm("s_bfe_i64 %0, %1, 0x1001b" : "=s"(keepJ[3]) : "s"(quad64) : "scc");
+  const bool endPartial = (c.quad & (1u << 27)) == 0u;
+  const uint32_t aLast = ldsBase + (c.aLast_kN & 0xffffu);
+  const uint32_t selC0 = c.selC0, selC1 = selC0 + 0x00020002u;
   const uint32_t selL0 = selC0 + 0x00010001u, selL1 = selL0 + 0x00020002u;
-  const bool rNear = sh <= 1;
-  const uint32_t rOff4 = rNear ? 0u : 4u;
-  const uint32_t selR0 = 0x0c000c00u + (uint32_t)(rNear ? sh + 3 : sh - 1) * 0x00010001u + 0x00010000u, selR1 = selR0 + 0x00020002u;
-  uint32_t* const dstc = cand + L.candOff + (long long)f * L.candCap + c.segOff;
-  const int segCap = (int)c.segCap;
+  const uint32_t rOff4 = (c.quad >> 26) & 4u;
+  const uint32_t selR0 = c.selR0, selR1 = selR0 + 0x00020002u;
+  uint32_t* const dstc =
+      reinterpret_cast<uint32_t*>(reinterpret_cast<uint8_t*>(cand) + (long long)(c.cand + (uint64_t)fu * c.candCap));
+  const int segCap = (int)((c.counts >> 10) & 0x7ffu);
   int nOut = 0;
   for (int pass = 0; pass < 2; pass++) {
     const int th = pass == 0 ? g.iniTh : g.minTh;
     const uint32_t thLo = (uint32_t)th, thHi = ((uint32_t)th << 16) | 0xffffu;
     const int thB = th + (int)FAST_PK_BIAS;
-    int nList = 0, nCorn = 0;
+    uint32_t ringTop = ringAddr, cornTop = cornAddr;
+    const uint32_t ringFull = ringAddr + 2u * 64u, cornEnd = cornAddr + 2u * FW_CORN;
     bool flat = pass == 0;
     short2v looseMax = {-0x8000, -0x8000};
-    auto flush = [&](const int cnt) {
+    auto flush = [&](auto whole) {
+      constexpr bool WHOLE = decltype(whole)::value;
       __builtin_amdgcn_wave_barrier();
-      const int keepN = nList - cnt;
-      uint32_t e = (uint32_t)fwLds16(ringLane)[keepN];
+      const uint32_t newTop = WHOLE ? ringTop - 2u * 64u : ringAddr;
+      uint32_t e = (uint32_t)fwLds16(newTop + 2u * (uint32_t)lane)[0];
       unsigned long long act = ~0ull;
-      if (cnt < 64) {
-        asm volatile("" ::: "memory");
+      if (!WHOLE) {
+        const int cnt = (int)((ringTop - ringAddr) >> 1);
         act = (1ull << cnt) - 1ull;
         e = lane < cnt ? e : eIdle;
       }
       const uint32_t sv = fwStrength<TS>(e);
-      const unsigned long long mc = __ballot((int)sv > thB) & act;
+      unsigned long long mc = __ballot((int)sv > thB);
+      if (!WHOLE) mc &= act;
       if (mc != 0ull) {
-        fwStoreB8(e + kS, sv, mc);
-        const int nc = (int)__popcll(mc);
-        if (nCorn + nc <= FW_CORN) fwStoreB16((cornAddr + 2u * (uint32_t)nCorn) + 2u * (uint32_t)fwMbcnt(mc), e, mc);
-        nCorn += nc;
-      }
-      nList = keepN;
+        fwStoreB8<TS + 1>(e + kN, sv, mc);
+        const uint32_t top = cornTop + 2u * (uint32_t)__popcll(mc);
+        if (top <= cornEnd) fwStoreB16(cornTop + 2u * (uint32_t)fwMbcnt(mc), e, mc);
+        cornTop = top;
+      }
+      ringTop = newTop;
     };
     {
       uint32_t pos = pos0;
-      for (int idx0 = 0; idx0 < nItems; idx0 += 64) {
+      auto step = [&](auto lastStep) {
+        constexpr bool LAST = decltype(lastStep)::value;
         uint32_t a = pos & 0xffffu;
-        const bool tail = idx0 + 64 > nItems;
-        if (tail) {
-          asm volatile("" ::: "memory");
-          a = min(a, aLast);
-        }
+        if (LAST) a = min(a, aLast);
         const fw_lds_u32* const pa = fwLds32(a);
         const uint32_t t0 = pa[1], t1 = pa[2];
         const uint32_t cM = pa[3 * (TS / 4)], c0 = pa[3 * (TS / 4) + 1], c1 = pa[3 * (TS / 4) + 2];
@@ -751,26 +757,30 @@
         if ((fwGtLo(dm, thLo) | fwGtHi(dm, thHi)) != 0ull) {
           flat = false;
           unsigned long long keepEnd = ~0ull;
-          if (nvLast < 4) keepEnd = ~__ballot(pos >= lastThr);
-          const unsigned long long live = tail ? (1ull << (nItems - idx0)) - 1ull : ~0ull;
-          const uint32_t q0 = a + (uint32_t)(sh + 1);
+          if (endPartial) keepEnd = ~__ballot(pos >= lastThr);
+          const uint32_t q0 = a + sh1;
 #pragma unroll
           for (int j = 0; j < 4; j++) {
             const uint32_t dj = __builtin_bit_cast(uint32_t, d[j >> 1]);
-            unsigned long long m = ((j & 1) ? fwGtHi(dj, thHi) : fwGtLo(dj, thLo)) & live;
-            if (j >= nvLast) m &= keepEnd;
+            unsigned long long m = (j & 1) ? fwGtHi(dj, thHi) : fwGtLo(dj, thLo);
+            if (LAST) m &= ~0ull >> tailShift;
+            if (j > 0) m &= keepEnd | keepJ[j];
             if (m != 0ull) {
-              fwStoreB16((ringAddr + 2u * (uint32_t)nList) + 2u * (uint32_t)fwMbcnt(m), q0 + (uint32_t)j, m);
-              nList += (int)__popcll(m);
+              fwStoreB16(ringTop + 2u * (uint32_t)fwMbcnt(m), q0 + (uint32_t)j, m);
+              ringTop += 2u * (uint32_t)__popcll(m);
             }
             if (j & 1)
-              while (nList >= 64) flush(64);
+              while (ringTop >= ringFull) flush(std::true_type{});
           }
         }
-        pos += dPos;
-        pos = min(pos, pos + wrapK);
-      }
-      if (nList > 0) flush(nList);
+        if (!LAST) {
+          pos += dPos;
+          pos = min(pos, pos + wrapK);
+        }
+      };
+      for (int i = nFull; i > 0; i--) step(std::false_type{});
+      step(std::true_type{});
+      if (ringTop != ringAddr) flush(std::false_type{});
     }
     __builtin_amdgcn_wave_barrier();
     auto nms = [&](const uint32_t eIn, const bool act) {
@@ -786,14 +796,20 @@
         const int o = (int)(e - tileAddr) + 3 * TS + 3;
         const int row = TS == 64 ? (o >> 6) : (int)(((uint32_t)o * 43691u) >> 21);
         static_assert(TS == 64 || TS == 48, "row split of a tile offset");
-        if (slot < segCap) dstc[slot] = packCand(o - row * TS + ox, row + oy, sv - 1);
+        if (slot < segCap) dstc[slot] = packCand(o - row * TS, row, sv - 1) + c.oxy;
       }
       nOut += (int)__popcll(mk);
     };
-    if (nCorn <= FW_CORN) {
+    if (cornTop <= cornEnd) {
+      const int nCorn = (int)((cornTop - cornAddr) >> 1);
       for (int e0 = 0; e0 < nCorn; e0 += 64) nms((uint32_t)fwLds16(cornAddr)[min(e0 + lane, FW_CORN - 1)], e0 + lane < nCorn);
     } else {
-      const uint32_t invw = c_inv20.v[iw];
+      uint32_t quadHere = c.quad;
+      int chHere = ch;
+      asm volatile("" : "+s"(quadHere), "+s"(chHere));
+      const int iw = 1 + (int)__popc((quadHere >> 25) & 7u) + 4 * (int)(((quadHere >> 21) & 15u) - 1u);
+      const int ih = chHere - 6;
+      const uint32_t invw = ((1u << 20) + (uint32_t)iw - 1u) / (uint32_t)iw;
       const int py0 = (int)(((uint32_t)lane * invw) >> 20), px0 = lane - py0 * iw;
       const int dpy = (int)((64u * invw) >> 20), dpx = 64 - dpy * iw;
       int px = px0;
@@ -801,7 +817,7 @@
       const int npix = iw * ih;
       for (int idx0 = 0; idx0 < npix; idx0 += 64) {
         const bool live = idx0 + lane < npix;
-        const int sv = live ? (int)fwLds8(e + kS)[0] : 0;
+        const int sv = live ? (int)fwLds8(e + kN)[TS + 1] : 0;
         const unsigned long long any = __ballot(sv > 0);
         if (any) nms(e, sv > 0);
         px += dpx;
@@ -815,7 +831,7 @@
       if (flat && (fwGtLo(lm, (uint32_t)g.minTh) | fwGtHi(lm, ((uint32_t)g.minTh << 16) | 0xffffu)) == 0ull) break;
     }
   }
-  if (lane == 0) *myCount = min(nOut, segCap);
+  if (lane == 0) *myCount() = min(nOut, segCap);
   __builtin_amdgcn_wave_barrier();
   }
 }
@@ -2811,14 +2827,13 @@
   if (waveOk && img0Aligned && cells && !small) {
     const int groups = ((g.nCellsTotal + FW_CPW - 1) / FW_CPW + 8 * FW_XK - 1) / (8 * FW_XK) * (8 * FW_XK);
     const int ts = waveOk == 2 ? 48 : 64;
-    const int tileBytes = ch * ts + 16, smapBytes = (ch - 6 + 2) * ts;
-    const size_t lds = (size_t)(16 + tileBytes + smapBytes + FW_RING * 2 + FW_CORN * 2);
+    const FastWaveLds lds = fastWaveLds(g, ts);
     if (ts == 48)
-      hipLaunchKernelGGL(k_fast_wave<48>, dim3(groups, nFrames, 1), dim3(64, 1, 1), lds, st, img0, img0FrameStride, pyr, g, cells,
-                         cand, cellCount, tileBytes, smapBytes);
+      hipLaunchKernelGGL(k_fast_wave<48>, dim3(groups, nFrames, 1), dim3(64, 1, 1), (size_t)lds.total, st, img0, img0FrameStride, pyr, g,
+                         cells, cand, cellCount, lds.tileBytes, lds.smapBytes);
     else
-      hipLaunchKernelGGL(k_fast_wave<64>, dim3(groups, nFrames, 1), dim3(64, 1, 1), lds, st, img0, img0FrameStride, pyr, g, cells,
-                         cand, cellCount, tileBytes, smapBytes);
+      hipLaunchKernelGGL(k_fast_wave<64>, dim3(groups, nFrames, 1), dim3(64, 1, 1), (size_t)lds.total, st, img0, img0FrameStride, pyr, g,
+                         cells, cand, cellCount, lds.tileBytes, lds.smapBytes);
     return hipGetLastError();
   }
   dim3 block(FAST_T, 1, 1), grid(g.nCellsTotal, nFrames, 1);
```

Result: faster. 549,700 (median of 6 runs) (+3.5%).
